# cortes-ciriano-lab/DeMethify

Measured on AMD Instinct MI355X. Metric: NMF update iters/sec (1e6 CpG x 256 samples x 16 types), higher is better.
Workload: dtype f64; 1 GPU; headline_1e6x256_12+4; N_cpg=1000000, S_samples=256, n_known=12, n_unknown=4, inner_iters=20, restarts=64, restart_seed=1 + k, restart_placement=k mod n_gpus, parallelism=restart-sharded x1

## Files before the change

demethify_amd/_lib.py:

```python
from __future__ import annotations

import ctypes as C
from pathlib import Path

LIB_PATH = Path(__file__).resolve().parent / "libdemethify_hip.so"

DMF_OK = 0
DMF_PTR_DEVICE = 1
DMF_INIT_IN_UNIT_RANGE = 4
DMF_SELECT_COUNTS_F32_EXACT, DMF_SELECT_PURITY, DMF_SELECT_ALPHA_OUTSIDE_UNIT, DMF_SELECT_V_UNALIGNED = 1, 2, 4, 8
DMF_SELECT_X16 = 16
DMF_COUNTS_F64 = 2
DMF_WLS_TARGET_V, DMF_WLS_TARGET_DV = 0, 1
DMF_WLS_F64_ARRAYS = 8
DMF_ERR_BAD_ARG, DMF_ERR_NONFINITE, DMF_ERR_UNSUPPORTED = 1, 4, 5
DMF_ERR_BAD_SHAPE = 2
DMF_GRAM_INTEGER, DMF_GRAM_FP64, DMF_GRAM_LAST = 0, 1, 2
DMF_ROUTE_SOLVER, DMF_ROUTE_UPDATE_U = 0, 1
MOMENTUM_SCALARS = ("a1", "a2", "l_w", "l_w_prev", "l_h", "l_h_prev", "dsq", "rt_norm2", "u_norm2", "cf", "cf_prev",
                    "iters", "done", "arrive", "mom_n", "mom_i")
REPORT_INTS = ("N", "S", "n_c", "ND", "SD", "N16", "plane_stride", "has_D16", "has_X16", "has_W16", "has_Dt8", "has_mask_bits",
               "rtp_width", "rtp_borrows_rt", "n_test", "d_f32_exact")
REPORT_DBLS = ("kDsq", "kRtSumsq", "kDmax", "kF32ResidualMax", "kIntCountMax", "kRtOutsideUnit", "x16_dev", "x16_sum")
PROBLEM_ARRAYS = {"V": 0, "D": 1, "Rt": 2, "Rtp": 3, "D16": 4, "X16": 5, "W16": 6, "Dt8": 7, "mask_bits": 8, "consts": 9}
DMF_MODE_PARTIAL = 0
DMF_MODE_UNSUPERVISED = 1
MAX_K = 64
SMALL_MAX_S, SMALL_MAX_K, SMALL_MAX_NU, SMALL_MAX_ELEMENTS = 64, 16, 4, 1 << 20
SVD_MAX_S, SVD_MAX_NC, SVD_MAX_RANK, SVD_MAX_LDS = 512, 64, 64, 160 * 1024


def svd_project_lds_bytes(n_samples, rank):
    return 8 * (n_samples * rank + 8 * ((n_samples + 63) // 64 * 64 + 16) + 512)


KERNEL_ROWPASS, KERNEL_GRAM, KERNEL_ALPHA, KERNEL_COST = 0, 1, 2, 3
KERNEL_FAMILIES = ("rowpass", "gram", "alpha", "cost")

_p = C.c_void_p
_i64 = C.c_int64
_dbl_p = C.POINTER(C.c_double)

SIGNATURES = {
    "dmf_status_string": (C.c_char_p, [C.c_int]),
    "dmf_last_error": (C.c_char_p, []),
    "dmf_abi_version": (C.c_int, []),
    "dmf_context_create": (C.c_int, [C.c_int, _p, C.POINTER(_p)]),
    "dmf_context_destroy": (C.c_int, [_p]),
    "dmf_context_synchronize": (C.c_int, [_p]),
    "dmf_context_set_profiling": (C.c_int, [_p, C.c_int]),
    "dmf_context_kernel_time": (C.c_int, [_p, C.c_int, _dbl_p, C.POINTER(_i64)]),
    "dmf_context_reset_kernel_time": (C.c_int, [_p]),
    "dmf_context_set_generic": (C.c_int, [_p, C.c_int]),
    "dmf_context_set_x16": (C.c_int, [_p, C.c_int]),
    "dmf_context_set_rowpass_pair": (C.c_int, [_p, C.c_int]),
    "dmf_context_set_rowpass_defer_c": (C.c_int, [_p, C.c_int]),
    "dmf_context_set_stop_confirmation": (C.c_int, [_p, C.c_int]),
    "dmf_problem_create": (C.c_int, [_p, _i64, _i64, _i64, _p, _p, _p, C.c_int, C.POINTER(_p)]),
    "dmf_problem_gather": (C.c_int, [_p, _p, _p, _i64, C.POINTER(_p)]),
    "dmf_problem_gather_device": (C.c_int, [_p, _p, _p, _i64, C.POINTER(_p)]),
    "dmf_problem_mask": (C.c_int, [_p, _p, _p, C.c_int, C.POINTER(_p)]),
    "dmf_solver_holdout_error": (C.c_int, [_p, _p, _dbl_p, C.POINTER(_i64)]),
    "dmf_problem_destroy": (C.c_int, [_p]),
    "dmf_problem_shape": (C.c_int, [_p, C.POINTER(_i64), C.POINTER(_i64), C.POINTER(_i64)]),
    "dmf_problem_gram_known": (C.c_int, [_p, _p, C.c_char_p, _i64]),
    "dmf_problem_report": (C.c_int, [_p, C.POINTER(_i64), _dbl_p]),
    "dmf_problem_copy_out": (C.c_int, [_p, C.c_int, _p, _i64]),
    "dmf_gram_i8_describe": (C.c_int, [_i64, _i64, _i64, _i64, C.c_int, C.c_char_p, _i64]),
    "dmf_solver_gram": (C.c_int, [_p, C.c_int, _p, C.c_char_p, _i64]),
    "dmf_solver_row_moments": (C.c_int, [_p, _p, C.c_char_p, _i64]),
    "dmf_solver_momentum_state": (C.c_int, [_p, _dbl_p, _p, _p]),
    "dmf_cost": (C.c_int, [_p, _p, _p, _i64, _p, C.c_int, _dbl_p]),
    "dmf_cost_describe": (C.c_int, [_i64, _i64, _i64, C.c_int, _i64, C.c_int, C.c_int, C.c_int, C.c_char_p, _i64]),
    "dmf_problem_cost_describe": (C.c_int, [_p, _p, _i64, C.c_char_p, _i64]),
    "dmf_project_simplex": (C.c_int, [_p, _p, _i64, _i64, C.c_double, C.c_int, _p]),
    "dmf_update_u": (C.c_int, [_p, _p, _p, _p, _p, _i64, _i64, C.c_int, C.c_int, _dbl_p, _p, _p]),
    "dmf_update_alpha": (C.c_int, [_p, _p, _p, _i64, _p, _p, _i64, C.c_int, _dbl_p, _p, _p]),
    "dmf_wls_intercept": (C.c_int, [_p, _p, _p, _i64, C.c_int, C.c_int, _p, C.POINTER(C.c_int)]),
    "dmf_wls_moments": (C.c_int, [_p, _p, _p, _i64, C.c_int, C.c_int, _p]),
    "dmf_nnls_normal": (C.c_int, [_p, _p, _p, _i64, _i64, _p, C.POINTER(C.c_int)]),
    "dmf_svd_gram": (C.c_int, [_p, _p, _p, C.c_int, _p, C.POINTER(_i64)]),
    "dmf_svd_factor": (C.c_int, [_p, _p, _p, _p, _i64, C.c_int, _p, C.POINTER(_p)]),
    "dmf_svd_finish": (C.c_int, [_p, _p, _i64, _i64, _p, _p, C.c_int, _p]),
    "dmf_percentile_axis0": (C.c_int, [_p, _p, _i64, _i64, _p, _i64, C.c_int, _p]),
    "dmf_nanpercentile_axis0": (C.c_int, [_p, _p, _i64, _i64, _p, _i64, C.c_int, _p]),
    "dmf_solver_create": (C.c_int, [_p, _p, _p, _p, _i64, C.c_int, C.c_int, C.POINTER(_p)]),
    "dmf_solver_set_purity": (C.c_int, [_p, _p, C.c_int]),
    "dmf_solver_step": (C.c_int, [_p, _i64, _i64, C.c_double, C.POINTER(_i64), C.POINTER(C.c_int)]),
    "dmf_solver_get": (C.c_int, [_p, C.c_int, _p, _p, _dbl_p, C.POINTER(_i64)]),
    "dmf_solver_match_components": (C.c_int, [_p, _p, _i64, _p, _p]),
    "dmf_solver_get_u_permuted": (C.c_int, [_p, C.POINTER(C.c_int32), _p]),
    "dmf_solver_get_u_by_row": (C.c_int, [_p, _p, _i64, C.POINTER(C.c_int32), _p]),
    "dmf_solver_cost": (C.c_int, [_p, _dbl_p]),
    "dmf_solver_cost_begin": (C.c_int, [_p]),
    "dmf_solver_cost_end": (C.c_int, [_p, _dbl_p]),
    "dmf_solver_destroy": (C.c_int, [_p]),
    "dmf_solver_describe": (C.c_int, [_p, _i64, C.c_char_p, _i64]),
    "dmf_select_describe": (C.c_int, [_i64, _i64, _i64, _i64, C.c_int, C.c_int, _i64, C.c_int, C.c_char_p, _i64]),
    "dmf_u_phase_describe": (C.c_int, [_i64, _i64, _i64, _i64, C.c_int, C.c_int, _i64, C.c_int, C.c_int, C.c_char_p, _i64]),
    "dmf_solver_u_phase_describe": (C.c_int, [_p, _i64, C.c_int, C.c_char_p, _i64]),
    "dmf_solver_stop_info": (C.c_int, [_p, C.POINTER(C.c_int), C.POINTER(_i64), C.POINTER(_i64), _dbl_p]),
    "dmf_solver_rowpass_launches": (C.c_int, [_p, C.POINTER(_i64), C.POINTER(_i64)]),
    "dmf_solver_rowpass_schedule_counts": (C.c_int, [_p, C.POINTER(_i64), C.POINTER(_i64), C.POINTER(_i64)]),
    "dmf_table_scan": (C.c_int, [C.c_char_p, C.c_char, C.POINTER(_i64), C.POINTER(C.c_int), C.POINTER(C.c_int),
                                 C.POINTER(C.c_int)]),
    "dmf_table_read": (C.c_int, [C.c_char_p, C.c_char, C.c_int, C.c_int, _i64, _p, _i64, C.c_double, _p, _i64, C.c_int]),
    "dmf_host_alloc": (_p, [C.c_size_t, C.POINTER(C.c_int)]),
    "dmf_host_free": (None, [_p, C.c_int]),
    "dmf_write_interval_csv": (C.c_int, [C.c_char_p, C.c_char_p, _p, _p, _i64, C.c_int, C.c_int, C.c_int]),
    "dmf_stage_upload": (C.c_int, [_p, _p, C.c_size_t, C.POINTER(C.c_void_p)]),
    "dmf_stage_free": (C.c_int, [_p, _p]),
    "dmf_stage_download": (C.c_int, [_p, _p, C.c_size_t, _p]),
    "dmf_mask_draw": (C.c_int, [_p, _p, C.POINTER(C.c_int), _i64, _i64, C.c_uint64, C.POINTER(C.c_void_p),
                                C.POINTER(_i64)]),
    "dmf_solve": (C.c_int, [_p, _p, _p, _p, _i64, C.c_int, _i64, _i64, C.c_double, C.c_int, _p, _p,
                            _dbl_p, C.POINTER(_i64)]),
    "dmf_solve_small_supported": (C.c_int, [_i64, _i64, _i64, _i64, C.c_int]),
    "dmf_solve_small": (C.c_int, [_p, _p, _i64, _p, _p, _p, _i64, C.c_int, _i64, _i64, C.c_double, _i64, C.c_int, _p, _p, _p, _p]),
    "dmf_solve_small_purity": (C.c_int, [_p, _p, _i64, _p, _p, _p, _p, _i64, C.c_int, _i64, _i64, C.c_double, _i64, C.c_int, _p, _p,
                                         _p, _p]),
}

_lib = None


class DemethifyHipError(RuntimeError):

    def __init__(self, status: int, where: str, detail: str = ""):
        self.status = status
        msg = f"{where}: status {status}"
        if detail:
            msg += f" ({detail})"
        super().__init__(msg)


def _preload_torch_hip_runtime():
    import importlib.util
    import os

# ... 48 lines not shown
```

demethify_amd/csrc/dmf_api.h:

```cpp
#pragma once
#include <hip/hip_runtime.h>

#include <cmath>
#include <cstdio>
#include <cstdlib>
#include <cstring>
#include <memory>
#include <mutex>
#include <new>
#include <unordered_map>
#include <utility>
#include <vector>

#include "../../include/demethify_hip.h"
#include "dmf_internal.h"
#include "dmf_select.h"

using dmf::SolverState;

namespace dmf_api {

int hip_fail(hipError_t e, const char* what, const char* file, int line);

#define HIP_TRY(expr)                                                                          \
    do {                                                                                       \
        hipError_t e_ = (expr);                                                                \
        if (e_ != hipSuccess) return dmf_api::hip_fail(e_, #expr, __FILE_NAME__, __LINE__);    \
    } while (0)

#define DMF_TRY(expr)                 \
    do {                              \
        int s_ = (expr);              \
        if (s_ != DMF_OK) return s_;  \
    } while (0)

constexpr int kEventPool = 2048;

struct FamilyClock {
    std::vector<hipEvent_t> start, stop;
    int used = 0;
    double total_ms = 0.0;
    int64_t launches = 0;
};

}

struct dmf_context {
    int device = 0;
    hipStream_t stream = nullptr;
    bool own_stream = false;
    unsigned profiling = 0;
    int stop_confirmation = 0;
    int generic_level = 0;
    bool x16 = true;
    bool rowpass_pair = true;
    bool rowpass_defer_c = true;
    double* scratch = nullptr;
    hipMemPool_t pool = nullptr;
    std::unordered_map<void*, size_t> live;
    std::unordered_map<size_t, std::vector<void*>> kept;
    size_t kept_bytes = 0;
    std::vector<hipEvent_t> events;
    std::vector<double*> pinned_moms;
    std::vector<void*> pinned_states;
    hipStream_t copy_stream = nullptr;
    std::mutex copy_mutex;
    dmf_api::FamilyClock clocks[DMF_KERNEL_FAMILIES];
};

namespace dmf_api {

hipError_t pool_alloc(dmf_context* ctx, void** p, size_t bytes);
void pool_free(dmf_context* ctx, void* p);
hipError_t stage_alloc(dmf_context* ctx, hipStream_t st, void** p, size_t bytes);
void stage_release(dmf_context* ctx, hipStream_t st, void* p);

template <class T>
class DevBuf {
  public:
    DevBuf() = default;
    DevBuf(DevBuf&& o) noexcept : ctx_(o.ctx_), ptr_(o.ptr_), owned_(o.owned_), stage_(o.stage_) {
        o.ptr_ = nullptr, o.owned_ = false;
    }
    DevBuf& operator=(DevBuf&& o) noexcept {
        if (this != &o) {
            reset();
            ctx_ = o.ctx_, ptr_ = o.ptr_, owned_ = o.owned_, stage_ = o.stage_;
            o.ptr_ = nullptr, o.owned_ = false;
        }
        return *this;
    }
    ~DevBuf() { reset(); }
    hipError_t alloc(dmf_context* ctx, size_t count) {
        reset();
        const hipError_t e = pool_alloc(ctx, (void**)&ptr_, count * sizeof(T));
        if (e != hipSuccess) ptr_ = nullptr;
        ctx_ = ctx, owned_ = e == hipSuccess, stage_ = nullptr;
        return e;
    }
    hipError_t alloc_staged(dmf_context* ctx, size_t count, hipStream_t st) {
        reset();
        const hipError_t e = stage_alloc(ctx, st, (void**)&ptr_, count * sizeof(T));
        if (e != hipSuccess) ptr_ = nullptr;
        ctx_ = ctx, owned_ = e == hipSuccess, stage_ = st;
        return e;
    }
    T* release() {
        T* p = ptr_;
        ptr_ = nullptr, owned_ = false;
        return p;
    }
    void borrow(const T* p) { reset(), ptr_ = const_cast<T*>(p); }
    void reset() {
        if (owned_ && stage_ != nullptr) stage_release(ctx_, stage_, ptr_);
        else if (owned_) pool_free(ctx_, ptr_);
        ptr_ = nullptr, owned_ = false;
    }
    T* get() const { return ptr_; }
    operator T*() const { return ptr_; }
    T* operator->() const { return ptr_; }

  private:
    dmf_context* ctx_ = nullptr;
    T* ptr_ = nullptr;
    bool owned_ = false;
    hipStream_t stage_ = nullptr;
};

enum ProblemConst { kDsq, kRtSumsq, kDmax, kF32ResidualMax, kIntCountMax, kRtOutsideUnit, kProblemConsts };

struct JobTable {
    std::vector<short> h_k, h_l;
    std::vector<int> h_dst;
    DevBuf<short> k, l;
    DevBuf<int> dst;
    int n = 0;
    template <class Keep>
    void build(int l_first, int l_last, Keep keep) {
        for (int ll = l_first; ll <= l_last; ++ll)
            for (int kk = 0; kk <= ll; ++kk) {
                if (!keep(kk, ll)) continue;
                h_k.push_back((short)kk);
                h_l.push_back((short)ll);
                h_dst.push_back(dmf::tri(kk, ll));
            }
        n = (int)h_k.size();
    }
    int upload(dmf_context* ctx) {
        HIP_TRY(k.alloc(ctx, n));
        HIP_TRY(l.alloc(ctx, n));
        HIP_TRY(dst.alloc(ctx, n));
        HIP_TRY(hipMemcpyAsync(k, h_k.data(), n * sizeof(short), hipMemcpyHostToDevice, ctx->stream));
        HIP_TRY(hipMemcpyAsync(l, h_l.data(), n * sizeof(short), hipMemcpyHostToDevice, ctx->stream));
        HIP_TRY(hipMemcpyAsync(dst, h_dst.data(), n * sizeof(int), hipMemcpyHostToDevice, ctx->stream));
        return DMF_OK;
    }
};

}

struct dmf_problem {
    dmf_context* ctx = nullptr;
    int64_t N = 0, S = 0, n_c = 0;
    dmf_api::DevBuf<double> V, D, Rt;
    dmf_api::DevBuf<double> Rtp;
    dmf_api::DevBuf<double> consts;
    double h_consts[dmf_api::kProblemConsts] = {};
    dmf_api::DevBuf<unsigned short> D16;
    dmf_api::DevBuf<signed char> Dt8;
    int ND = 0;
    int SD = 0;
    int64_t N16 = 0, plane_stride = 0;
    dmf_api::DevBuf<unsigned short> X16;
    double x16_dev = 0.0, x16_sum = 0.0;
    bool d_f32_exact = false;
    dmf_api::DevBuf<double> gb_known;
    dmf::GramRan known_ran;
    dmf_api::DevBuf<unsigned char> mask_bits;
    dmf_api::DevBuf<unsigned short> W16;
    int64_t n_test = 0;
    dmf::ProblemView view() const {
        dmf::ProblemView v;
        v.V = V, v.D = D, v.D16 = D16, v.X16 = X16, v.Dt8 = Dt8;
        v.plane_stride = plane_stride, v.SD = SD, v.ND = ND;
        v.Rt = Rt, v.Rtp = Rtp;
        v.N = N, v.S = (int)S, v.n_c = (int)n_c;
        return v;
    }
};

constexpr size_t kPinnedStateBytes = (sizeof(SolverState) + 15) / 16 * 16 + 16;

struct dmf_solver {
    dmf_context* ctx = nullptr;
    const dmf_problem* p = nullptr;
    int64_t n_u = 0;
    int mode = 0;
    dmf::ShapeKey key;
    dmf::PathSpec spec;
    dmf_api::DevBuf<double> cm;
    dmf_api::DevBuf<double> beta_tab;
    int64_t beta_cap = 0;
    dmf_api::DevBuf<long long> slab_i8;
    int64_t slab_i8_words = 0;
    dmf_api::DevBuf<long long> acc_i8;
    dmf_api::DevBuf<double> purity;
    dmf_api::DevBuf<double> u2_partials;
    dmf_api::DevBuf<double> u, u_prev, u_next;
    dmf_api::DevBuf<double> alpha, alpha_prev;
    dmf_api::DevBuf<double> gb;
    dmf::GramRan last_gram;
    int last_gram_source = -1;
    dmf_api::DevBuf<double> slab;
    int64_t slab_doubles = 0;
    dmf_api::DevBuf<double> partials;
    dmf_api::DevBuf<SolverState> state;
    SolverState* h_state = nullptr;
    dmf_api::JobTable jobs;
    bool cf_pending = true;
    double* mom_host = nullptr;
    dmf_api::DevBuf<double> mom_dev;
    hipEvent_t cost_event = nullptr;
    bool cost_pending = false;
    bool in_flight = false;
    bool confirm_stops = false;
    double cf_stream = 0.0;
    long long cf_stream_iter = -1;
    long long n_rowpass = 0, n_rowpass_pair = 0;
    long long n_rowpass_defer = 0;
    long long n_confirmed = 0, n_unconfirmed = 0;
    dmf::IterateView iterate() const {
        dmf::IterateView it;
        it.u = u, it.u_prev = u_prev, it.alpha = alpha, it.state = state;
        it.n_u = (int)n_u, it.mode = mode;
        return it;
    }
    dmf::AlphaView alpha_view() const {
        dmf::AlphaView a;
        a.gb = gb, a.alpha = alpha, a.alpha_prev = alpha_prev, a.purity = purity, a.state = state, a.partials = partials;
        a.S = (int)p->S, a.n_c = (int)p->n_c, a.n_u = (int)n_u;
        return a;
    }
    dmf::UScratch scratch() const {
        dmf::UScratch sc;
        sc.cm = cm, sc.beta = beta_tab, sc.slab = slab, sc.u2_partials = u2_partials;
        return sc;
    }
};

namespace dmf_api {

struct HandleDeleter {
    void operator()(dmf_problem* p) const { dmf_problem_destroy(p); }
    void operator()(dmf_solver* s) const { dmf_solver_destroy(s); }
};
using ProblemPtr = std::unique_ptr<dmf_problem, HandleDeleter>;
using SolverPtr = std::unique_ptr<dmf_solver, HandleDeleter>;

int clock_drain(dmf_context* ctx, FamilyClock& c);

struct FamilyScope {
    dmf_context* ctx;
    FamilyClock* c = nullptr;
    int slot = -1;
    FamilyScope(dmf_context* ctx_, int family) : ctx(ctx_) {
        if (!((ctx->profiling >> family) & 1u)) return;
        c = &ctx->clocks[family];
        if (c->start.empty()) {
            c->start.resize(kEventPool);
            c->stop.resize(kEventPool);
            for (int i = 0; i < kEventPool; ++i) {
                hipEventCreateWithFlags(&c->start[i], hipEventDisableSystemFence);
                hipEventCreateWithFlags(&c->stop[i], hipEventDisableSystemFence);
            }
        }
        if (c->used == kEventPool) clock_drain(ctx, *c);
        slot = c->used++;
        hipEventRecord(c->start[slot], ctx->stream);
    }
    ~FamilyScope() {
        if (c != nullptr) hipEventRecord(c->stop[slot], ctx->stream);
    }
};

int check_ctx(dmf_context* ctx);

template <class T>
int import_array(dmf_context* ctx, const void* src, size_t count, int flags, DevBuf<T>& dst) {
    dst.reset();
    if (count == 0) return DMF_OK;
    if (flags & DMF_PTR_DEVICE) {
        dst.borrow(static_cast<const T*>(src));
        return DMF_OK;
    }
    HIP_TRY(dst.alloc(ctx, count));
    HIP_TRY(hipMemcpyAsync(dst, src, count * sizeof(T), hipMemcpyHostToDevice, ctx->stream));
    HIP_TRY(hipStreamSynchronize(ctx->stream));
    return DMF_OK;
}
int export_array(dmf_context* ctx, const void* dev_src, size_t bytes, int flags, void* dst);

hipError_t enqueue_cost(dmf_context* ctx, const dmf::ProblemView& p, const double* u, const double* alpha, int n_u,
                        double* scratch, double* out);
bool cost_reads_u16_only(dmf_context* ctx, const dmf::ProblemView& p, int n_u);
int cost_to_host(dmf_context* ctx, const dmf::ProblemView& p, const double* u, const double* alpha, int n_u,
                 double* host_slot, bool wait);

int enqueue_u_phase(dmf_solver* s, int n_iter2, dmf::RowKind row);
dmf::RowKind standalone_row_kind(const dmf_solver* s, int n_iter2);
int enqueue_gram(dmf_solver* s, dmf::GramKind kind, bool heed_done = true, dmf::GramRan* ran = nullptr);
dmf::GramKind fp64_gram_kind(const dmf_solver* s);
int enqueue_alpha_phase(dmf_solver* s, dmf::AlphaKind kind, int n_iter2);
// ... 5 lines not shown
```

demethify_amd/csrc/dmf_api_context.hip:

```cpp
#include "dmf_api.h"

namespace dmf_api {

static thread_local char g_last_error[512] = "";

int hip_fail(hipError_t e, const char* what, const char* file, int line) {
    snprintf(g_last_error, sizeof(g_last_error), "%s failed at %s:%d: %s", what, file, line, hipGetErrorString(e));
    return DMF_ERR_HIP;
}

int clock_drain(dmf_context* ctx, FamilyClock& c) {
    if (c.used == 0) return DMF_OK;
    HIP_TRY(hipStreamSynchronize(ctx->stream));
    for (int i = 0; i < c.used; ++i) {
        float ms = 0.f;
        HIP_TRY(hipEventElapsedTime(&ms, c.start[i], c.stop[i]));
        c.total_ms += ms;
    }
    c.launches += c.used;
    c.used = 0;
    return DMF_OK;
}

static bool pool_enabled() {
// ... 218 lines not shown
    HIP_TRY(state.alloc_staged(ctx, kStateWords, st));
    uint32_t h_state[kStateWords] = {};
    std::memcpy(h_state, key, 624 * sizeof(uint32_t));
    HIP_TRY(hipMemcpyAsync(state, h_state, sizeof(h_state), hipMemcpyHostToDevice, st));
    HIP_TRY(dmf::launch_mask_draw(state, *pos, N, S, threshold, bits, reinterpret_cast<unsigned long long*>(state + 624), st));
    HIP_TRY(hipMemcpyAsync(h_state, state, sizeof(h_state), hipMemcpyDeviceToHost, st));
    HIP_TRY(hipStreamSynchronize(st));
    unsigned long long result[2];
    std::memcpy(result, h_state + 624, sizeof(result));
    std::memcpy(key, h_state, 624 * sizeof(uint32_t));
    *pos = (int)result[1];
    *n_kept = (int64_t)result[0];
    *out_bits = bits.release();
    return DMF_OK;
}

int dmf_stage_free(dmf_context* ctx, void* dev) {
    if (ctx == nullptr) return DMF_ERR_BAD_ARG;
    if (dev == nullptr) return DMF_OK;
    HIP_TRY(hipSetDevice(ctx->device));
    pool_free(ctx, dev);
    return DMF_OK;
}

int dmf_context_synchronize(dmf_context* ctx) {
    DMF_TRY(check_ctx(ctx));
    HIP_TRY(hipStreamSynchronize(ctx->stream));
    return DMF_OK;
}

int dmf_context_set_profiling(dmf_context* ctx, int enabled) {
    DMF_TRY(check_ctx(ctx));
    if (!enabled)
        for (auto& c : ctx->clocks) DMF_TRY(clock_drain(ctx, c));
    ctx->profiling = enabled == 0 ? 0u : enabled == 1 ? ~0u : (unsigned)enabled >> 1;
    return DMF_OK;
}

int dmf_context_kernel_time(dmf_context* ctx, int family, double* total_ms, int64_t* launches) {
    DMF_TRY(check_ctx(ctx));
    if (family < 0 || family >= DMF_KERNEL_FAMILIES) return DMF_ERR_BAD_ARG;
    FamilyClock& c = ctx->clocks[family];
    DMF_TRY(clock_drain(ctx, c));
    if (total_ms) *total_ms = c.total_ms;
    if (launches) *launches = c.launches;
    return DMF_OK;
}

int dmf_context_reset_kernel_time(dmf_context* ctx) {
    DMF_TRY(check_ctx(ctx));
    for (auto& c : ctx->clocks) {
        DMF_TRY(clock_drain(ctx, c));
        c.total_ms = 0.0;
        c.launches = 0;
    }
    return DMF_OK;
}

int dmf_context_set_generic(dmf_context* ctx, int enabled) {
    if (ctx == nullptr) return DMF_ERR_BAD_ARG;
    if (enabled < 0 || enabled > 4) return DMF_ERR_BAD_ARG;
    ctx->generic_level = enabled;
    return DMF_OK;
}

int dmf_context_set_x16(dmf_context* ctx, int enabled) {
    if (ctx == nullptr || enabled < 0 || enabled > 1) return DMF_ERR_BAD_ARG;
    ctx->x16 = enabled != 0;
    return DMF_OK;
}

int dmf_context_set_rowpass_pair(dmf_context* ctx, int enabled) {
    if (ctx == nullptr || enabled < 0 || enabled > 1) return DMF_ERR_BAD_ARG;
    ctx->rowpass_pair = enabled != 0;
    return DMF_OK;
}

int dmf_context_set_rowpass_defer_c(dmf_context* ctx, int enabled) {
    if (ctx == nullptr || enabled < 0 || enabled > 1) return DMF_ERR_BAD_ARG;
    ctx->rowpass_defer_c = enabled != 0;
    return DMF_OK;
}

int dmf_context_set_stop_confirmation(dmf_context* ctx, int mode) {
    if (ctx == nullptr || mode < 0 || mode > 2) return DMF_ERR_BAD_ARG;
    ctx->stop_confirmation = mode;
    return DMF_OK;
}

}
```

demethify_amd/csrc/dmf_api_problem.hip:

```cpp
#include "dmf_api.h"

namespace dmf_api {

static int alloc_count_copies(dmf_problem* p, int ND, bool x16, bool w16) {
    dmf_context* ctx = p->ctx;
    p->ND = ND;
    p->SD = (int)((p->S + 63) / 64 * 64);
    p->N16 = (p->N + 15) / 16 * 16;
    p->plane_stride = ((p->N + 31) / 32) * (p->SD / 32) * 1024;
    const size_t u16_elems = (size_t)p->N16 * p->SD;
    HIP_TRY(p->D16.alloc(ctx, u16_elems));
    HIP_TRY(p->Dt8.alloc(ctx, (size_t)p->plane_stride * ND));
    if (x16) HIP_TRY(p->X16.alloc(ctx, u16_elems));
    if (w16) HIP_TRY(p->W16.alloc(ctx, u16_elems));
    return DMF_OK;
}

static void known_route(dmf_problem* p, const char* piece) {
    char* t = p->known_ran.text;
    const size_t have = std::strlen(t), cap = sizeof(p->known_ran.text);
    snprintf(t + have, cap - have, "%s%s", have > 0 ? " " : "", piece);
}

static int problem_finalize(dmf_problem* p, bool counts_done = false) {
    dmf_context* ctx = p->ctx;
    const int64_t N = p->N, S = p->S, n_c = p->n_c;
    double* const h = p->h_consts;
    HIP_TRY(p->consts.alloc(ctx, kProblemConsts));
    if (!counts_done) HIP_TRY(dmf::launch_max_f64(p->D, N * S, ctx->scratch, p->consts + kDmax, ctx->stream));
    if (n_c > 0) {
        HIP_TRY(dmf::launch_sumsq_f64(p->Rt, N * n_c, ctx->scratch + 1024, p->consts + kRtSumsq, nullptr, ctx->stream));
    } else {
        HIP_TRY(hipMemsetAsync(p->consts + kRtSumsq, 0, sizeof(double), ctx->stream));
    }
    if (!counts_done) {
        HIP_TRY(dmf::launch_f32_residual_max(p->D, N * S, ctx->scratch + 2048, p->consts + kF32ResidualMax, ctx->stream));
        HIP_TRY(dmf::launch_int_count_max(p->D, N * S, ctx->scratch + 3072, p->consts + kIntCountMax, ctx->stream));
        if (n_c > 0) {
            HIP_TRY(dmf::launch_unit_range_check(p->Rt, N * n_c, ctx->scratch, p->consts + kRtOutsideUnit, ctx->stream));
        } else {
            HIP_TRY(hipMemsetAsync(p->consts + kRtOutsideUnit, 0, sizeof(double), ctx->stream));
        }
    }
    {
        double got[kProblemConsts];
        HIP_TRY(hipMemcpyAsync(got, p->consts, sizeof(got), hipMemcpyDeviceToHost, ctx->stream));
        HIP_TRY(hipStreamSynchronize(ctx->stream));
        h[kRtSumsq] = got[kRtSumsq];
        if (!counts_done)
            for (int i = kDmax; i < kProblemConsts; ++i) h[i] = got[i];
    }
    h[kDsq] = h[kDmax] * h[kDmax];
    p->d_f32_exact = h[kF32ResidualMax] == 0.0;
    HIP_TRY(hipMemcpyAsync(p->consts, h, kProblemConsts * sizeof(double), hipMemcpyHostToDevice, ctx->stream));
    HIP_TRY(hipStreamSynchronize(ctx->stream));
    if (!std::isfinite(h[kDmax]) || !std::isfinite(h[kRtSumsq])) return DMF_ERR_NONFINITE;

    if (!counts_done && ctx->generic_level == 0 && h[kIntCountMax] <= 32639.0 && h[kRtOutsideUnit] == 0.0 && S >= 2 &&
        S <= 2048 && n_c <= 48) {
        DMF_TRY(alloc_count_copies(p, h[kIntCountMax] <= 127.0 ? 1 : 2, ctx->x16, false));
        DevBuf<unsigned long long> x_stats;
        if (ctx->x16) HIP_TRY(x_stats.alloc(ctx, 3));
        HIP_TRY(dmf::launch_build_counts_int(p->D, p->V, N, (int)S, p->ND, p->D16, p->X16, p->N16, p->SD, p->Dt8,
                                             p->plane_stride, x_stats, ctx->stream));
        if (p->X16 != nullptr) {
            unsigned long long got[3] = {1, 0, 0};
            HIP_TRY(hipMemcpyAsync(got, x_stats, sizeof(got), hipMemcpyDeviceToHost, ctx->stream));
            HIP_TRY(hipStreamSynchronize(ctx->stream));
            if (got[0] != 0) {
                p->X16.reset();
            } else {
                std::memcpy(&p->x16_dev, &got[1], sizeof(double));
                p->x16_sum = (double)got[2];
            }
        }
    }

    if (n_c > 0 && n_c <= 48) {
        const int nct = (int)((n_c + 3) / 4 * 4);
        if (nct == n_c) {
            p->Rtp.borrow(p->Rt);
        } else {
            HIP_TRY(p->Rtp.alloc(ctx, (size_t)N * nct));
            HIP_TRY(dmf::launch_pad_rows(p->Rt, p->Rtp, N, (int)n_c, nct, ctx->stream));
        }
    }

    const dmf::ProblemView pv = p->view();
    JobTable jobs;
    jobs.build(0, (int)n_c, [](int, int) { return true; });
    const int n_jobs = jobs.n;
    const bool mfma = n_c >= 1 && ctx->generic_level != 1 && ctx->generic_level != 2;
    const int n_fast = mfma ? n_jobs - 1 : 0, n_dense = (int)(n_c * (n_c + 1) / 2);
    const bool int_known = mfma && ctx->generic_level == 0 && p->Dt8 != nullptr && p->D16 != nullptr && p->Rtp != nullptr &&
                           (reinterpret_cast<uintptr_t>(p->Rtp.get()) & 15) == 0 &&
                           dmf::gram_i8_known_supported((int)n_c, p->ND, N, p->SD);
    int64_t slab_doubles = dmf::gram_slab_doubles(N, (int)S, mfma ? 1 : n_jobs);
    if (mfma && !int_known) {
        const int64_t need = dmf::gram_mfma_slab_doubles(N, (int)S, n_fast);
        if (need > slab_doubles) slab_doubles = need;
    }
    DevBuf<double> slab, slab_bu;
    DevBuf<long long> slab_i8, acc;
    HIP_TRY(p->gb_known.alloc(ctx, (size_t)n_jobs * S));
    DMF_TRY(jobs.upload(ctx));
    HIP_TRY(slab.alloc(ctx, (size_t)slab_doubles));
    bool vdv_done = true;
    if (int_known) {
        const int64_t slab_words = dmf::gram_i8_slab_words_nf(N, p->SD, n_dense);
        const int64_t acc_words = dmf::gram_i8_acc_words_nf((int)S, n_dense, (int)n_c + 1);
        HIP_TRY(slab_i8.alloc(ctx, (size_t)slab_words));
        HIP_TRY(acc.alloc(ctx, (size_t)acc_words));
        HIP_TRY(slab_bu.alloc(ctx, (size_t)dmf::bu_cols_grid(N) * (n_c + 1) * S));
        HIP_TRY(hipMemsetAsync(acc, 0, (size_t)acc_words * sizeof(long long), ctx->stream));
        int ny = 0, n_slabs = 0;
        dmf::GramRan ran;
        HIP_TRY(dmf::launch_gram_i8(pv, nullptr, 0, jobs.k, jobs.l, n_dense, slab_i8, slab_words, nullptr, &ny, ctx->stream, &ran));
        known_route(p, "int_known");
        known_route(p, ran.text);
        HIP_TRY(dmf::launch_bu_cols(pv, p->Rt, (int)n_c, slab_bu, nullptr, &n_slabs, ctx->stream, &vdv_done));
        known_route(p, vdv_done ? "+ k_bu_cols2 with vDv" : "+ k_bu_cols");
        HIP_TRY(dmf::launch_gram_v2_reduce(slab_i8, ny, n_dense, p->SD, slab_bu, n_slabs, (int)n_c + (vdv_done ? 1 : 0), (int)S,
                                           acc, jobs.dst, p->gb_known, nullptr, nullptr, 0, nullptr, ctx->stream));
    } else if (mfma) {
        dmf::GramJobTable fast{jobs.k, jobs.l, jobs.dst, n_fast};
        int ny = 0;
        dmf::GramRan ran;
        HIP_TRY(dmf::launch_gram_mfma(pv, nullptr, 0, fast, n_dense, slab, slab_doubles, nullptr, &ny, ctx->stream, &ran));
        known_route(p, "fp64");
        known_route(p, ran.text);
        HIP_TRY(dmf::launch_gram_reduce(slab, ny, n_fast, (int)S, jobs.dst, p->gb_known, nullptr, ctx->stream));
    }
    if (int_known && vdv_done) {
    } else if (n_jobs - n_fast == 1 && ctx->generic_level != 1 && ctx->generic_level != 2 &&
               (int64_t)dmf::vdv_cols_grid(N) * S <= slab_doubles) {
        HIP_TRY(dmf::launch_vdv_cols(pv, slab, p->gb_known + (int64_t)jobs.h_dst[n_jobs - 1] * S, ctx->stream));
        known_route(p, p->known_ran.text[0] == 0 ? "fp64 k_vdv_cols" : "+ k_vdv_cols");
    } else {
        dmf::GramJobTable rest{jobs.k + n_fast, jobs.l + n_fast, jobs.dst + n_fast, n_jobs - n_fast};
        dmf::GramRan ran;
        if (p->known_ran.text[0] == 0) known_route(p, "fp64");
        else known_route(p, "+");
        HIP_TRY(dmf::launch_gram(pv, nullptr, 0, rest, slab, slab_doubles, p->gb_known, nullptr, ctx->stream, &ran));
        known_route(p, ran.text);
    }
    HIP_TRY(hipStreamSynchronize(ctx->stream));
    return DMF_OK;
}

static dmf::CostPlan cost_plan_of(dmf_context* ctx, const dmf::ProblemView& p, int n_u) {
    return dmf::cost_plan(dmf::cost_key(p, n_u, ctx->generic_level));
}

hipError_t enqueue_cost(dmf_context* ctx, const dmf::ProblemView& p, const double* u, const double* alpha, int n_u,
                        double* scratch, double* out) {
    return dmf::launch_cost_plan(cost_plan_of(ctx, p, n_u), p, u, alpha, n_u, scratch, out, ctx->stream);
}

bool cost_reads_u16_only(dmf_context* ctx, const dmf::ProblemView& p, int n_u) { return cost_plan_of(ctx, p, n_u).d16; }
// ... 148 lines not shown
    const bool x16 = ints && src->X16 != nullptr && ctx->x16;
    if (ints) DMF_TRY(alloc_count_copies(p.get(), src->ND, x16, true));
    DevBuf<unsigned long long> d_stats;
    HIP_TRY(d_stats.alloc(ctx, 3));
    HIP_TRY(dmf::launch_mask_problem(src->V, src->D, ints ? src->D16.get() : nullptr, x16 ? src->X16.get() : nullptr,
                                     p->mask_bits, p->V, p->D, p->D16, p->X16, p->W16, N, p->N16, (int)S, p->SD, d_stats,
                                     ctx->stream));
    if (ints) HIP_TRY(dmf::launch_build_dt8(p->D16, N, p->SD, p->ND, p->Dt8, p->plane_stride, ctx->stream));
    unsigned long long h_stats[3] = {0, 0, 0};
    HIP_TRY(hipMemcpyAsync(h_stats, d_stats, sizeof(h_stats), hipMemcpyDeviceToHost, ctx->stream));
    HIP_TRY(hipStreamSynchronize(ctx->stream));
    d_stats.reset();
    double dmax;
    std::memcpy(&dmax, &h_stats[0], sizeof(dmax));
    p->h_consts[kDmax] = dmax;
    p->h_consts[kF32ResidualMax] = src->h_consts[kF32ResidualMax];
    p->h_consts[kIntCountMax] = std::isfinite(src->h_consts[kIntCountMax]) ? dmax : src->h_consts[kIntCountMax];
    p->h_consts[kRtOutsideUnit] = src->h_consts[kRtOutsideUnit];
    p->x16_dev = x16 ? src->x16_dev : 0.0;
    p->x16_sum = (double)h_stats[1];
    p->n_test = (int64_t)h_stats[2];
    DMF_TRY(problem_finalize(p.get(), true));
    *out = p.release();
    return DMF_OK;
}

int dmf_problem_destroy(dmf_problem* p) {
    if (p == nullptr) return DMF_OK;
    hipSetDevice(p->ctx->device);
    delete p;
    return DMF_OK;
}

int dmf_problem_cost_describe(dmf_context* ctx, const dmf_problem* p, int64_t n_u, char* buf, int64_t cap) {
    if (ctx == nullptr || p == nullptr || buf == nullptr || cap < 1 || n_u < 0 || p->ctx != ctx) return DMF_ERR_BAD_ARG;
    if (p->n_c + n_u < 1 || p->n_c + n_u > dmf::kMaxK) return DMF_ERR_BAD_ARG;
    dmf::describe_cost_plan(cost_plan_of(ctx, p->view(), (int)n_u), buf, (size_t)cap);
    return DMF_OK;
}

int dmf_problem_gram_known(const dmf_problem* p, double* out, char* out_text, int64_t cap) {
    if (p == nullptr || out == nullptr || (out_text != nullptr && cap < 1)) return DMF_ERR_BAD_ARG;
    dmf_context* ctx = p->ctx;
    DMF_TRY(check_ctx(ctx));
    const size_t n = (size_t)(p->n_c + 1) * (p->n_c + 2) / 2 * p->S;
    HIP_TRY(hipMemcpyAsync(out, p->gb_known, n * sizeof(double), hipMemcpyDeviceToHost, ctx->stream));
    HIP_TRY(hipStreamSynchronize(ctx->stream));
    if (out_text != nullptr) snprintf(out_text, (size_t)cap, "%s", p->known_ran.text);
    return DMF_OK;
}

int dmf_problem_report(const dmf_problem* p, int64_t* out_ints, double* out_dbls) {
    if (p == nullptr || out_ints == nullptr || out_dbls == nullptr) return DMF_ERR_BAD_ARG;
    const int64_t rtp_width = p->Rtp != nullptr ? (p->n_c + 3) / 4 * 4 : 0;
    const int64_t ints[DMF_REPORT_INTS] = {p->N, p->S, p->n_c, p->ND, p->SD, p->N16, p->plane_stride,
                                           p->D16 != nullptr, p->X16 != nullptr, p->W16 != nullptr, p->Dt8 != nullptr,
                                           p->mask_bits != nullptr, rtp_width,
                                           p->Rtp != nullptr && p->Rtp.get() == p->Rt.get(), p->n_test, p->d_f32_exact};
    std::memcpy(out_ints, ints, sizeof(ints));
    for (int i = 0; i < kProblemConsts; ++i) out_dbls[i] = p->h_consts[i];
    out_dbls[kProblemConsts] = p->x16_dev;
    out_dbls[kProblemConsts + 1] = p->x16_sum;
    return DMF_OK;
}

int dmf_problem_copy_out(const dmf_problem* p, int which, void* out, int64_t bytes) {
    if (p == nullptr || out == nullptr) return DMF_ERR_BAD_ARG;
    dmf_context* ctx = p->ctx;
    DMF_TRY(check_ctx(ctx));
    const size_t elems = (size_t)p->N * p->S, u16_bytes = (size_t)p->N16 * p->SD * sizeof(unsigned short);
    const void* src = nullptr;
    size_t size = 0;
    switch (which) {
        case DMF_ARRAY_V: src = p->V, size = elems * sizeof(double); break;
        case DMF_ARRAY_D: src = p->D, size = elems * sizeof(double); break;
        case DMF_ARRAY_RT: src = p->Rt, size = (size_t)p->N * p->n_c * sizeof(double); break;
        case DMF_ARRAY_RTP: src = p->Rtp, size = (size_t)p->N * ((p->n_c + 3) / 4 * 4) * sizeof(double); break;
        case DMF_ARRAY_D16: src = p->D16, size = u16_bytes; break;
        case DMF_ARRAY_X16: src = p->X16, size = u16_bytes; break;
        case DMF_ARRAY_W16: src = p->W16, size = u16_bytes; break;
        case DMF_ARRAY_DT8: src = p->Dt8, size = (size_t)p->plane_stride * p->ND; break;
        case DMF_ARRAY_MASK_BITS: src = p->mask_bits, size = (size_t)p->N * (size_t)((p->S + 7) / 8); break;
        case DMF_ARRAY_CONSTS: src = p->consts, size = kProblemConsts * sizeof(double); break;
        default: return DMF_ERR_BAD_ARG;
    }
    if (src == nullptr || size == 0) return DMF_ERR_BAD_ARG;
    if (bytes < 0 || (size_t)bytes != size) return DMF_ERR_BAD_SHAPE;
    return export_array(ctx, src, size, 0, out);
}

int dmf_problem_shape(const dmf_problem* p, int64_t* N, int64_t* S, int64_t* n_c) {
    if (p == nullptr) return DMF_ERR_BAD_ARG;
    if (N) *N = p->N;
    if (S) *S = p->S;
    if (n_c) *n_c = p->n_c;
    return DMF_OK;
}

}
```

demethify_amd/csrc/dmf_api_solver.hip:

```cpp
#include "dmf_api.h"

namespace dmf_api {

using dmf::kSplitInnerSteps;

static int ensure_split_scratch(dmf_solver* s, int n_iter2) {
    dmf_context* ctx = s->ctx;
    if (s->cm == nullptr) HIP_TRY(s->cm.alloc(ctx, (size_t)dmf::u_phase_split_cm_doubles(s->p->N, (int)s->n_u)));
    if (s->beta_cap < n_iter2 || s->beta_tab == nullptr) {
        s->beta_cap = n_iter2 > 0 ? n_iter2 : 1;
        HIP_TRY(s->beta_tab.alloc(ctx, (size_t)s->beta_cap));
    }
    return DMF_OK;
}

int enqueue_u_phase(dmf_solver* s, int n_iter2, dmf::RowKind row) {
    dmf_context* ctx = s->ctx;
    const dmf::ProblemView pv = s->p->view();
    FamilyScope scope(ctx, DMF_KERNEL_ROWPASS);
    switch (row) {
        case dmf::RowKind::CmI8InnerRows:
            DMF_TRY(ensure_split_scratch(s, n_iter2));
            HIP_TRY(dmf::launch_u_phase_split_i8(pv, s->iterate(), n_iter2, s->scratch(), ctx->stream));
            return DMF_OK;
// ... 41 lines not shown
    return b;
}

static int gram_i8_and_reduce(dmf_solver* s, const GramI8Buffers& b, int n_slabs, const double* u2_partials, int n_u2,
                              dmf::GramRan* ran = nullptr) {
    dmf_context* ctx = s->ctx;
    const dmf_problem* p = s->p;
    const int S = (int)p->S, n_c = (int)p->n_c, n_u = (int)s->n_u, nf = n_c * n_u + n_u * (n_u + 1) / 2;
    int ny = 0;
    HIP_TRY(dmf::launch_gram_i8(p->view(), s->u, n_u, s->jobs.k, s->jobs.l, nf, b.slab_i8, b.slab_i8_words, b.done, &ny,
                                ctx->stream, ran));
    HIP_TRY(dmf::launch_gram_v2_reduce(b.slab_i8, ny, nf, p->SD, b.slab_bu, n_slabs, n_u, S, b.acc, s->jobs.dst, b.gb, b.done,
                                       u2_partials, n_u2, s->state, ctx->stream));
    return DMF_OK;
}

static int gram_bu_cols_i8(dmf_solver* s, const GramI8Buffers& b, dmf::GramRan* ran = nullptr) {
    int n_slabs = 0;
    HIP_TRY(dmf::launch_bu_cols(s->p->view(), s->u, (int)s->n_u, b.slab_bu, b.done, &n_slabs, s->ctx->stream));
    return gram_i8_and_reduce(s, b, n_slabs, nullptr, 0, ran);
}

int enqueue_gram(dmf_solver* s, dmf::GramKind kind, bool heed_done, dmf::GramRan* ran) {
    dmf_context* ctx = s->ctx;
    const dmf::ProblemView pv = s->p->view();
    const int S = pv.S, n_u = (int)s->n_u;
    const int* done = heed_done ? &s->state->done : nullptr;
    FamilyScope scope(ctx, DMF_KERNEL_GRAM);
    if (kind == dmf::GramKind::BuColsI8) {
        GramI8Buffers b = solver_i8_buffers(s);
        b.done = done;
        return gram_bu_cols_i8(s, b, ran);
    }
    if (kind == dmf::GramKind::GramU) {
        int ny = 0;
        HIP_TRY(dmf::launch_gram_u(pv, s->u, n_u, s->slab, done, &ny, ctx->stream, ran));
        HIP_TRY(dmf::launch_gram_reduce(s->slab, ny, s->jobs.n, S, s->jobs.dst, s->gb, done, ctx->stream));
        return DMF_OK;
    }
    dmf::GramJobTable jobs{s->jobs.k, s->jobs.l, s->jobs.dst, s->jobs.n};
    if (kind == dmf::GramKind::GramMfma) {
        int ny = 0;
        HIP_TRY(dmf::launch_gram_mfma(pv, s->u, n_u, jobs, s->jobs.n - n_u, s->slab, s->slab_doubles, done, &ny, ctx->stream, ran));
        HIP_TRY(dmf::launch_gram_reduce(s->slab, ny, s->jobs.n, S, s->jobs.dst, s->gb, done, ctx->stream));
        return DMF_OK;
    }
    HIP_TRY(dmf::launch_gram(pv, s->u, n_u, jobs, s->slab, s->slab_doubles, s->gb, done, ctx->stream, ran));
    return DMF_OK;
}

dmf::GramKind fp64_gram_kind(const dmf_solver* s) {
    return s->spec.use_gram_spec ? dmf::GramKind::GramU : s->spec.use_gram_mfma ? dmf::GramKind::GramMfma : dmf::GramKind::Gram;
}

int enqueue_alpha_phase(dmf_solver* s, dmf::AlphaKind kind, int n_iter2) {
    FamilyScope scope(s->ctx, DMF_KERNEL_ALPHA);
    HIP_TRY(dmf::launch_alpha(kind, s->alpha_view(), n_iter2, s->ctx->stream));
    return DMF_OK;
}

constexpr int kLastGramI8Tail = 100, kLastGramFused = 101;
static dmf::GramRan* last_gram_slot(dmf_solver* s, int source) {
    if (s->last_gram_source == source) return nullptr;
    s->last_gram_source = source;
    return &s->last_gram;
}

static int enqueue_gram_i8_tail(dmf_solver* s, dmf::AlphaKind alpha, int n_iter2, int grid) {
    {
        FamilyScope scope(s->ctx, DMF_KERNEL_GRAM);
        DMF_TRY(gram_i8_and_reduce(s, solver_i8_buffers(s), grid, s->u2_partials, grid, last_gram_slot(s, kLastGramI8Tail)));
    }
    return enqueue_alpha_phase(s, alpha, n_iter2);
}

static int enqueue_outer_iteration(dmf_solver* s, int n_iter2) {
    dmf_context* ctx = s->ctx;
    s->in_flight = true;
    const dmf_problem* p = s->p;
    const int S = (int)p->S;
    const dmf::IterationPlan plan = dmf::plan_iteration(s->key, s->spec, n_iter2, s->purity != nullptr);
    if (plan.row == dmf::RowKind::RowpassV2) {
        int grid = 0;
        bool paired = false, deferred = false;
        {
            FamilyScope scope(ctx, DMF_KERNEL_ROWPASS);
            dmf::ProblemView pv = p->view();
            if (!s->key.x16) pv.X16 = nullptr;
            HIP_TRY(dmf::launch_rowpass_v2(pv, s->iterate(), n_iter2, s->scratch(), &grid, s->key.rowpass_pair, &paired,
                                           s->key.rowpass_defer_c && s->key.x_byte, &deferred, ctx->stream));
            ++s->n_rowpass;
            s->n_rowpass_pair += paired ? 1 : 0;
            s->n_rowpass_defer += deferred ? 1 : 0;
        }
        return enqueue_gram_i8_tail(s, plan.alpha, n_iter2, grid);
    }
    if (plan.row == dmf::RowKind::CmI8InnerBu) {
        int grid = 0;
        DMF_TRY(ensure_split_scratch(s, n_iter2));
        {
            FamilyScope scope(ctx, DMF_KERNEL_ROWPASS);
            HIP_TRY(dmf::launch_u_phase_split_i8_bu(p->view(), s->iterate(), n_iter2, s->scratch(), &grid, ctx->stream));
        }
        return enqueue_gram_i8_tail(s, plan.alpha, n_iter2, grid);
    }
    if (plan.row == dmf::RowKind::RowpassFused) {
        const int64_t n_full = p->N - (p->N & 15), n_tail = p->N - n_full;
        const dmf::ProblemView pv = p->view();
        int grid = 0, ny_tail = 0;
        {
            FamilyScope scope(ctx, DMF_KERNEL_ROWPASS);
            HIP_TRY(dmf::launch_rowpass_fused(pv.rows(0, n_full), s->iterate(), n_iter2, s->scratch(), &grid, ctx->stream));
        }
        if (n_tail > 0) {
            const dmf::ProblemView tail = pv.rows(n_full, n_tail);
            const dmf::IterateView it_tail = s->iterate().rows(n_full);
            HIP_TRY(dmf::launch_u_phase_mfma(tail, it_tail, n_iter2, ctx->stream));
            HIP_TRY(dmf::launch_sumsq_f64(it_tail.u, n_tail * s->n_u, ctx->scratch, s->u2_partials + grid, &s->state->done,
                                          ctx->stream));
            HIP_TRY(dmf::launch_gram_u(tail, it_tail.u, it_tail.n_u, s->slab + (int64_t)2 * grid * s->jobs.n * S,
                                       &s->state->done, &ny_tail, ctx->stream));
        }
        if (dmf::GramRan* ran = last_gram_slot(s, kLastGramFused))
            snprintf(ran->text, sizeof(ran->text), "k_rowpass_fused<%d,%d> phase C slabs=%d%s", (int)(p->n_c + 3) / 4, (int)s->n_u,
                     2 * grid, n_tail > 0 ? " + k_gram_u tail" : "");
        HIP_TRY(dmf::launch_finish_u_norm(s->u2_partials, grid + (n_tail > 0 ? 1 : 0), s->state, ctx->stream));
        {
            FamilyScope scope(ctx, DMF_KERNEL_GRAM);
            HIP_TRY(dmf::launch_gram_reduce(s->slab, 2 * grid + ny_tail, s->jobs.n, S, s->jobs.dst, s->gb,
                                            &s->state->done, ctx->stream));
        }
        return enqueue_alpha_phase(s, plan.alpha, n_iter2);
    }
    DMF_TRY(enqueue_u_phase(s, n_iter2, plan.row));
    HIP_TRY(dmf::launch_sumsq_f64(s->u, p->N * s->n_u, ctx->scratch, &s->state->u_norm2, &s->state->done,
                                  ctx->stream));
    HIP_TRY(dmf::launch_set_lh(s->state, ctx->stream));
    DMF_TRY(enqueue_gram(s, plan.gram, true, last_gram_slot(s, (int)plan.gram)));
    return enqueue_alpha_phase(s, plan.alpha, n_iter2);
}

int fetch_state(dmf_solver* s) {
    HIP_TRY(hipMemcpyAsync(s->h_state, s->state, sizeof(SolverState), hipMemcpyDeviceToHost, s->ctx->stream));
    HIP_TRY(hipStreamSynchronize(s->ctx->stream));
    s->in_flight = false;
    return DMF_OK;
}

int push_state(dmf_solver* s) {
    HIP_TRY(hipMemcpyAsync(s->state, s->h_state, sizeof(SolverState), hipMemcpyHostToDevice, s->ctx->stream));
    HIP_TRY(hipStreamSynchronize(s->ctx->stream));
    return DMF_OK;
}

constexpr int kMomRows = 64, kMomSteps = 64;

__global__ void k_set_momentum(SolverState* state, const double* mom, int stride, int rows, int n) {
    state->mom = mom;
    state->mom_stride = stride;
    state->mom_rows = rows;
    state->mom_i = 0;
    state->mom_n = n;
}

static double momentum_advance(double& a) {
#pragma clang fp contract(off)
    const double a0 = a;
    const double sq = 4.0 * a0 * a0;
    a = (1.0 + std::sqrt(1.0 + sq)) / 2.0;
    return (a0 - 1.0) / a;
}

static int upload_momentum_rows(dmf_solver* s, int rows, int n) {
    dmf_context* ctx = s->ctx;
    const int stride = 2 + 2 * n;
    if (s->mom_host == nullptr) {
        if (!ctx->pinned_moms.empty()) {
            s->mom_host = ctx->pinned_moms.back();
            ctx->pinned_moms.pop_back();
        } else {
            HIP_TRY(hipHostMalloc((void**)&s->mom_host, (size_t)kMomRows * (2 + 2 * kMomSteps) * sizeof(double)));
        }
        HIP_TRY(s->mom_dev.alloc(ctx, (size_t)kMomRows * (2 + 2 * kMomSteps)));
    }
    double a1 = s->h_state->a1, a2 = s->h_state->a2;
    for (int r = 0; r < rows; ++r) {
        double* row = s->mom_host + (size_t)r * stride;
        for (int t = 0; t < n; ++t) {
            row[2 + t] = momentum_advance(a1);
            row[2 + n + t] = momentum_advance(a2);
        }
        row[0] = a1;
        row[1] = a2;
    }
    HIP_TRY(hipMemcpyAsync(s->mom_dev, s->mom_host, (size_t)rows * stride * sizeof(double), hipMemcpyHostToDevice, ctx->stream));
    hipLaunchKernelGGL(k_set_momentum, dim3(1), dim3(1), 0, ctx->stream, s->state.get(), (const double*)s->mom_dev.get(), stride,
                       rows, n);
    HIP_TRY(hipGetLastError());
    return DMF_OK;
}

__global__ void k_set_tol(SolverState* state, double tol, double band) {
    state->tol = tol;
    state->band = band;
}

constexpr double kConfirmBand = 10.0;
constexpr double kGramCostRelErr = 1e-15;

static double* cost_slot(const dmf_solver* s) {
    return reinterpret_cast<double*>(reinterpret_cast<char*>(s->h_state) + kPinnedStateBytes - 16);
}

static int solver_setup(dmf_solver* s, const double* u0, const double* alpha0, int flags) {
    dmf_context* ctx = s->ctx;
    const dmf_problem* p = s->p;
    const int64_t N = p->N, S = p->S, n_c = p->n_c, n_u = s->n_u, K = n_c + n_u;
    dmf::ShapeKey& key = s->key;
    key.N = N;
    key.S = (int)S;
    key.n_c = (int)n_c;
    key.n_u = (int)n_u;
    key.nd = (p->ND > 0 && p->D16 != nullptr) ? p->ND : 0;
    key.SD = p->SD;
    key.x16 = key.nd > 0 && p->X16 != nullptr;
    key.rowpass_pair = ctx->rowpass_pair;
    key.rowpass_defer_c = ctx->rowpass_defer_c;
    key.x_byte = key.x16 && p->h_consts[kIntCountMax] <= 255.0;
    key.level = ctx->generic_level;
    key.d_f32_exact = p->d_f32_exact;
    key.rtp_present = n_c == 0 || p->Rtp != nullptr;
    key.v_align = (unsigned)(reinterpret_cast<uintptr_t>(p->V.get()) & 15);
    key.rtp_align = (unsigned)(reinterpret_cast<uintptr_t>(p->Rtp.get()) & 15);
    key.alpha_unit = true;
    s->spec = dmf::select_path(key);
    if ((s->spec.use_v2 || s->spec.use_cm_i8) && !(flags & DMF_INIT_IN_UNIT_RANGE)) {
        bool in_unit = true;
        if (flags & DMF_PTR_DEVICE) {
            double outside = 0.0;
            HIP_TRY(dmf::launch_unit_range_check(alpha0, K * S, ctx->scratch, ctx->scratch + 2048, ctx->stream));
            HIP_TRY(hipMemcpyAsync(&outside, ctx->scratch + 2048, sizeof(double), hipMemcpyDeviceToHost, ctx->stream));
            HIP_TRY(hipStreamSynchronize(ctx->stream));
            in_unit = outside == 0.0;
        } else {
            for (int64_t i = 0; i < K * S; ++i)
                if (!(alpha0[i] >= 0.0 && alpha0[i] <= 1.0)) {
                    in_unit = false;
                    break;
                }
        }
        if (!in_unit) {
            key.alpha_unit = false;
            s->spec = dmf::select_path(key);
        }
    }
    if (!s->spec.supported) return DMF_ERR_UNSUPPORTED;
    s->in_flight = true;
    s->jobs.build((int)n_c, (int)K, [n_c, K](int k, int l) {
        if (l == (int)K && k < (int)n_c) return false;
        return !(l == (int)K && k == (int)K);
    });
    const int n_jobs = s->jobs.n;
    s->slab_doubles = dmf::gram_slab_doubles(N, (int)S, n_jobs);
    if (s->spec.use_gram_spec) {
        const int64_t spec = dmf::gram_u_slab_doubles(N, (int)S, (int)n_c, (int)n_u);
        if (spec > s->slab_doubles) s->slab_doubles = spec;
    }
    if (s->spec.use_gram_mfma) {
        const int64_t need = dmf::gram_mfma_slab_doubles(N, (int)S, n_jobs);
        if (need > s->slab_doubles) s->slab_doubles = need;
    }
    if (s->spec.use_fused) {
        const int64_t spec = dmf::rowpass_fused_slab_doubles(N - (N & 15), (int)S, (int)n_c, (int)n_u) +
                             dmf::gram_u_slab_doubles(16, (int)S, (int)n_c, (int)n_u);
        if (spec > s->slab_doubles) s->slab_doubles = spec;
    }
    if (s->spec.use_v2) {
        const int64_t bu = (int64_t)dmf::rowpass_v2_grid(N, (int)S) * n_u * S;
        if (bu > s->slab_doubles) s->slab_doubles = bu;
    }
    if (s->spec.use_gram_i8) {
        const int64_t bu = (int64_t)dmf::bu_cols_grid(N) * n_u * S;
        if (bu > s->slab_doubles) s->slab_doubles = bu;
        if (s->spec.use_cm_i8) {
            const int64_t bu2 = (int64_t)dmf::u_inner_bu_grid(N, (int)S) * n_u * S;
            if (bu2 > s->slab_doubles) s->slab_doubles = bu2;
        }
    }
    const size_t un = (size_t)N * n_u, an = (size_t)K * S;
    const size_t un_alloc = (un + 1) & ~(size_t)1;
    const size_t gbn = (size_t)(K + 1) * (K + 2) / 2 * S;
    const int nb_alpha = (int)((S + 63) / 64);
    HIP_TRY(s->u.alloc(ctx, un_alloc));
    HIP_TRY(s->u_prev.alloc(ctx, un_alloc));
    if (s->spec.u_path == 2) HIP_TRY(s->u_next.alloc(ctx, un_alloc));
    HIP_TRY(s->alpha.alloc(ctx, an));
    HIP_TRY(s->alpha_prev.alloc(ctx, an));
    HIP_TRY(s->gb.alloc(ctx, gbn));
    HIP_TRY(s->slab.alloc(ctx, (size_t)s->slab_doubles));
    HIP_TRY(s->partials.alloc(ctx, (size_t)2 * (nb_alpha + S)));
    HIP_TRY(s->u2_partials.alloc(ctx, 4096));
    if (s->spec.use_v2 || s->spec.use_gram_i8) {
        s->slab_i8_words = dmf::gram_i8_slab_words(N, p->SD, (int)n_c, (int)n_u);
        HIP_TRY(s->slab_i8.alloc(ctx, (size_t)s->slab_i8_words));
        const size_t acc_words = (size_t)dmf::gram_i8_acc_words((int)S, (int)n_c, (int)n_u);
        HIP_TRY(s->acc_i8.alloc(ctx, acc_words));
        HIP_TRY(hipMemsetAsync(s->acc_i8, 0, acc_words * sizeof(long long), ctx->stream));
    }
    HIP_TRY(s->state.alloc(ctx, 1));
    if (!ctx->pinned_states.empty()) {
// ... 277 lines not shown
    if (s->h_state->done != 0) return DMF_ERR_BAD_ARG;
    dmf::CmRan ran;
    s->in_flight = true;
    const int status = solver_row_moments_enqueue(s, row, out_cm, &ran);
    if (status != DMF_OK) (void)hipStreamSynchronize(ctx->stream);
    s->in_flight = false;
    if (status == DMF_OK && out_text != nullptr) snprintf(out_text, (size_t)cap, "%s", ran.text);
    return status;
}

int dmf_solver_momentum_state(const dmf_solver* s, double* scalars, double* alpha_prev, double* u_prev) {
    if (s == nullptr || scalars == nullptr) return DMF_ERR_BAD_ARG;
    dmf_context* ctx = s->ctx;
    DMF_TRY(check_ctx(ctx));
    const dmf_problem* p = s->p;
    SolverState st;
    HIP_TRY(hipMemcpyAsync(&st, s->state.get(), sizeof(SolverState), hipMemcpyDeviceToHost, ctx->stream));
    if (alpha_prev != nullptr)
        HIP_TRY(hipMemcpyAsync(alpha_prev, s->alpha_prev.get(), (size_t)(p->n_c + s->n_u) * p->S * sizeof(double), hipMemcpyDeviceToHost,
                               ctx->stream));
    if (u_prev != nullptr)
        HIP_TRY(hipMemcpyAsync(u_prev, s->u_prev.get(), (size_t)p->N * s->n_u * sizeof(double), hipMemcpyDeviceToHost, ctx->stream));
    HIP_TRY(hipStreamSynchronize(ctx->stream));
    const double out[DMF_MOMENTUM_SCALARS] = {st.a1, st.a2, st.l_w, st.l_w_prev, st.l_h, st.l_h_prev, st.dsq, st.rt_norm2,
                                              st.u_norm2, st.cf, st.cf_prev, (double)st.iters, (double)st.done,
                                              (double)st.arrive, (double)st.mom_n, (double)st.mom_i};
    for (int i = 0; i < DMF_MOMENTUM_SCALARS; ++i) scalars[i] = out[i];
    return DMF_OK;
}

int dmf_solver_destroy(dmf_solver* s) {
    if (s == nullptr) return DMF_OK;
    dmf_context* ctx = s->ctx;
    hipSetDevice(ctx->device);
    if (s->cost_pending) (void)hipEventSynchronize(s->cost_event);
    if (s->in_flight) (void)hipStreamSynchronize(ctx->stream);
    if (s->cost_event) ctx->events.push_back(s->cost_event);
    if (s->mom_host) ctx->pinned_moms.push_back(s->mom_host);
    if (s->h_state) ctx->pinned_states.push_back(s->h_state);
    delete s;
    return DMF_OK;
}

int dmf_solver_describe(const dmf_solver* s, int64_t n_iter2, char* buf, int64_t cap) {
    if (s == nullptr || buf == nullptr || cap < 1 || n_iter2 < 0) return DMF_ERR_BAD_ARG;
    const dmf::IterationPlan plan = dmf::plan_iteration(s->key, s->spec, (int)n_iter2, s->purity != nullptr);
    dmf::describe_plan(s->key, plan, buf, (size_t)cap);
    return DMF_OK;
}

int dmf_solver_u_phase_describe(const dmf_solver* s, int64_t n_iter2, int route, char* buf, int64_t cap) {
    if (s == nullptr || buf == nullptr || cap < 1 || n_iter2 < 0 || n_iter2 > (1 << 20) ||
        (route != DMF_ROUTE_SOLVER && route != DMF_ROUTE_UPDATE_U))
        return DMF_ERR_BAD_ARG;
    dmf::describe_u_phase(s->key, s->spec, (int)n_iter2, s->purity != nullptr, route == DMF_ROUTE_UPDATE_U, buf, (size_t)cap);
    return DMF_OK;
}

int dmf_solver_stop_info(const dmf_solver* s, int* confirm_stops, int64_t* n_confirmed, int64_t* n_unconfirmed,
                         double* last_stream_cost) {
    if (s == nullptr) return DMF_ERR_BAD_ARG;
    if (confirm_stops) *confirm_stops = s->confirm_stops ? 1 : 0;
    if (n_confirmed) *n_confirmed = s->n_confirmed;
    if (n_unconfirmed) *n_unconfirmed = s->n_unconfirmed;
    if (last_stream_cost) *last_stream_cost = s->cf_stream_iter >= 0 ? s->cf_stream : std::nan("");
    return DMF_OK;
}

int dmf_solver_rowpass_launches(const dmf_solver* s, int64_t* total, int64_t* paired) {
    if (s == nullptr) return DMF_ERR_BAD_ARG;
    if (total) *total = s->n_rowpass;
    if (paired) *paired = s->n_rowpass_pair;
    return DMF_OK;
}

int dmf_solver_rowpass_schedule_counts(const dmf_solver* s, int64_t* total, int64_t* paired, int64_t* deferred) {
    if (s == nullptr) return DMF_ERR_BAD_ARG;
    if (total) *total = s->n_rowpass;
    if (paired) *paired = s->n_rowpass_pair;
    if (deferred) *deferred = s->n_rowpass_defer;
    return DMF_OK;
}

int dmf_solve(dmf_context* ctx, const dmf_problem* p, const double* u0, const double* alpha0, int64_t n_u,
              int mode, int64_t n_iter1, int64_t n_iter2, double tol, int flags, double* out_u,
              double* out_alpha, double* out_cost, int64_t* out_iters) {
    dmf_solver* raw = nullptr;
    DMF_TRY(dmf_solver_create(ctx, p, u0, alpha0, n_u, mode, flags, &raw));
    SolverPtr s(raw);
    DMF_TRY(dmf_solver_step(raw, n_iter1, n_iter2, tol, nullptr, nullptr));
    return dmf_solver_get(raw, flags, out_u, out_alpha, out_cost, out_iters);
}

}
```

demethify_amd/csrc/dmf_internal.h:

```cpp
#pragma once
#include <hip/hip_runtime.h>
#include <stdint.h>

#include "dmf_select.h"

namespace dmf {

struct SolverState {
    double a1;
    double a2;
    double l_w;
    double l_w_prev;
    double l_h;
    double l_h_prev;
    double dsq;
    double rt_norm2;
    double u_norm2;
    double cf;
    double cf_prev;
    double tol;
    long long iters;
    double band;
    int done;
    int arrive;
    const double* mom;
    int mom_stride, mom_rows, mom_i, mom_n;
};

__device__ __forceinline__ const double* momentum_row(const SolverState* __restrict__ state, int n_iter2) {
    return (state->mom != nullptr && state->mom_n == n_iter2 && state->mom_i < state->mom_rows)
               ? state->mom + (int64_t)state->mom_i * state->mom_stride
               : nullptr;
}

__host__ __device__ inline int tri(int k, int l) { return l * (l + 1) / 2 + k; }

constexpr int kMaxK = 64;
constexpr int kGramChunk = 16;
constexpr int kRowsPerBlockU = 64;

struct GramJobTable {
    const short* k_idx;
    const short* l_idx;
    const int* dst_row;
    int count;
};

struct PercentilePlan {
    long long k_prev, k_next;
    double gamma;
    int from_top;
    int pad;
};

struct ProblemView {
    const double* V = nullptr;
    const double* D = nullptr;
    const unsigned short* D16 = nullptr;
    const unsigned short* X16 = nullptr;
    const signed char* Dt8 = nullptr;
    int64_t plane_stride = 0;
    int SD = 0, ND = 0;
    const double* Rt = nullptr;
    const double* Rtp = nullptr;
    int64_t N = 0;
    int S = 0, n_c = 0;
    unsigned v_align() const { return (unsigned)(reinterpret_cast<uintptr_t>(V) & 15); }
    ProblemView rows(int64_t first, int64_t count) const {
        ProblemView r;
        r.V = V + first * S;
        r.D = D + first * S;
        r.Rt = Rt ? Rt + first * n_c : nullptr;
        r.Rtp = Rtp ? Rtp + first * ((n_c + 3) / 4 * 4) : nullptr;
        r.N = count;
        r.S = S;
        r.n_c = n_c;
        return r;
    }
};

struct IterateView {
    double* u = nullptr;
    double* u_prev = nullptr;
    const double* alpha = nullptr;
    SolverState* state = nullptr;
    int n_u = 0, mode = 0;
    IterateView rows(int64_t first) const {
        IterateView r = *this;
        r.u = u + first * n_u;
        r.u_prev = u_prev + first * n_u;
        return r;
    }
};

struct AlphaView {
    const double* gb = nullptr;
    double* alpha = nullptr;
    double* alpha_prev = nullptr;
    const double* purity = nullptr;
    SolverState* state = nullptr;
    double* partials = nullptr;
    int S = 0, n_c = 0, n_u = 0;
};

struct UScratch {
    double* cm = nullptr;
    double* beta = nullptr;
    double* slab = nullptr;
    double* u2_partials = nullptr;
};


hipError_t launch_convert_counts(const long long* src, double* dst, int64_t n, hipStream_t st);
hipError_t launch_max_f64(const double* x, int64_t n, double* scratch, double* out, hipStream_t st);
hipError_t launch_f32_residual_max(const double* x, int64_t n, double* scratch, double* out, hipStream_t st);
hipError_t launch_int_count_max(const double* x, int64_t n, double* scratch, double* out, hipStream_t st);
hipError_t launch_unit_range_check(const double* x, int64_t n, double* scratch, double* out, hipStream_t st);
hipError_t launch_sumsq_f64(const double* x, int64_t n, double* scratch, double* out,
                            const int* done_flag, hipStream_t st);
hipError_t launch_pad_rows(const double* src, double* dst, int64_t n_rows, int width_src, int width_dst,
                           hipStream_t st);
hipError_t launch_index_range_check(const long long* idx, int64_t n_idx, int64_t n_src, unsigned int* flag, hipStream_t st);
hipError_t launch_gather_rows(const double* src, double* dst, const long long* idx, int64_t n_idx,
                              int64_t width, hipStream_t st);

inline CostKey cost_key(const ProblemView& p, int n_u, int level) {
    CostKey k;
    k.S = p.S, k.n_c = p.n_c, k.n_u = n_u;
    k.d16 = p.D16 != nullptr;
    k.SD = p.SD;
    k.v_align = p.v_align();
    k.rtp_present = p.Rtp != nullptr;
    k.level = level;
    return k;
}
hipError_t launch_cost_plan(const CostPlan& plan, const ProblemView& p, const double* u, const double* alpha, int n_u,
                            double* scratch, double* out, hipStream_t st);
int vdv_cols_grid(int64_t N);
hipError_t launch_vdv_cols(const ProblemView& p, double* slab, double* out, hipStream_t st);

struct GramRan {
    char text[192] = "";
// ... 62 lines not shown

hipError_t launch_alpha(AlphaKind kind, const AlphaView& a, int n_iter2, hipStream_t st);
hipError_t launch_set_lh(SolverState* state, hipStream_t st);
hipError_t launch_project_simplex(const double* X, double* out, int K, int S, double z,
                                  hipStream_t st);
hipError_t launch_scatter_known_block(const double* gb_known, double* gb, int n_c, int K, int S,
                                      hipStream_t st);
hipError_t launch_init_state(SolverState* state, const double* consts, const double* alpha,
                             int S, int n_c, int n_u, hipStream_t st);

int64_t u_phase_split_cm_doubles(int64_t N, int n_u);
hipError_t launch_u_phase_split(const ProblemView& p, const IterateView& it, int n_iter2, const UScratch& scratch,
                                hipStream_t st);

bool cm_i8_supported(unsigned v_align, int S, int n_c, int n_u, int ND, int SD);
struct CmI8Launch {
    int mt0 = 0, mt1 = 0;
    int c_tile = 0, c_store = 0;
    size_t lds = 0;
    int grid = 0;
    int64_t blocks_per_wave = 0;
};
struct CmI8Panel {
    int col0 = 0, Sp = 0;
    bool s4 = false;
    int ncgx = 2;
    int tpl = 0;
    int n_launch = 0;
    CmI8Launch first, last;
};
constexpr int kCmMaxPanels = 8;
struct CmI8Plan {
    bool supported = false;
    int64_t N = 0;
    int S = 0, n_c = 0, n_u = 0;
    int nkc = 0, nd = 1;
    int nmt = 0, n_ct = 0;
    int n_panels = 0;
    CmI8Panel panel[kCmMaxPanels];
};
CmI8Plan cm_i8_plan(int64_t N, int S, int n_c, int n_u, int ND);
CmI8Launch cm_i8_launch_of(const CmI8Plan& g, int panel, int li);
int describe_cm_i8_plan(const CmI8Plan& g, char* buf, size_t cap);
struct CmRan {
    char text[2048] = "";
};
hipError_t launch_cm_i8(const ProblemView& p, const IterateView& it, double* cm, hipStream_t st, CmRan* ran = nullptr);
hipError_t launch_u_phase_split_i8(const ProblemView& p, const IterateView& it, int n_iter2, const UScratch& scratch,
                                   hipStream_t st);

bool u_inner_bu_supported(unsigned v_align, int S, int SD, int n_u, int n_iter2);
int u_inner_bu_grid(int64_t N, int S);
hipError_t launch_u_phase_split_i8_bu(const ProblemView& p, const IterateView& it, int n_iter2, const UScratch& scratch,
                                      int* grid_out, hipStream_t st);

bool u_phase_big_supported(int S, int n_c, int n_u, int n_iter2);
hipError_t launch_u_phase_big(const ProblemView& p, const IterateView& it, int n_iter2, hipStream_t st);

hipError_t launch_gram_mfma(const ProblemView& p, const double* u, int n_u, GramJobTable jobs, int n_dense, double* slab,
                            int64_t slab_doubles, const int* done_flag, int* ny_out, hipStream_t st, GramRan* ran = nullptr);
int64_t gram_mfma_slab_doubles(int64_t N, int S, int n_jobs);

hipError_t launch_gather_counts_int(const unsigned short* src16, const unsigned short* src_x16, const long long* idx,
                                    int64_t n_idx, int SD, int ND, unsigned short* D16, unsigned short* X16, int64_t N16,
                                    signed char* Dt8, int64_t plane_stride, unsigned int* max_out,
                                    unsigned long long* xsum_out, hipStream_t st);
constexpr double kX16MaxDev = 8.0 * 0x1p-53;
hipError_t launch_build_counts_int(const double* D, const double* V, int64_t N, int S, int ND, unsigned short* D16,
                                   unsigned short* X16, int64_t N16, int SD, signed char* Dt8, int64_t plane_stride,
                                   unsigned long long* x_stats, hipStream_t st);
hipError_t launch_build_dt8(const unsigned short* D16, int64_t N, int SD, int ND, signed char* Dt8, int64_t plane_stride,
                            hipStream_t st);
hipError_t launch_mask_problem(const double* srcV, const double* srcD, const unsigned short* src16,
                               const unsigned short* srcX, const unsigned char* bits, double* dstV, double* dstD,
                               unsigned short* dst16, unsigned short* dstX, unsigned short* W16, int64_t N, int64_t N16, int S,
                               int SD, unsigned long long* stats, hipStream_t st);
hipError_t launch_holdout_weights_f64(const unsigned char* bits, double* W, int64_t N, int S, hipStream_t st);
constexpr int64_t kMaskDrawMaxS = ((int64_t)1 << 31) - 1, kMaskDrawMaxElements = (int64_t)1 << 60;
hipError_t launch_mask_draw(unsigned int* key_io, int pos, int64_t N, int64_t S, unsigned long long threshold,
                            unsigned char* bits, unsigned long long* result, hipStream_t st);
bool rowpass_v2_supported(int S, int n_c, int n_u, int n_iter2);
int rowpass_v2_grid(int64_t N, int S);
hipError_t launch_rowpass_v2(const ProblemView& p, const IterateView& it, int n_iter2, const UScratch& scratch, int* grid_out,
                             bool pair, bool* paired_out, bool defer_c, bool* deferred_out, hipStream_t st);
bool rowpass_v2_pair_fits(int S, int n_u, int n_iter2);
bool gram_i8_supported(int n_c, int n_u, int ND, int64_t N, int SD);
struct GramI8Plan {
    bool supported = false;
    int xl = 1, nd = 1, ring = 8;
    int nf = 0, launches = 0;
    int nsh = 0, ny = 0;
    int64_t rows_per_wg = 0;
    int blocks = 0, last = 0;
    int tail = 0;
    bool xcd = false;
};
GramI8Plan gram_i8_plan(int64_t N, int SD, int n_c, int n_u, int ND);
void describe_gram_i8_plan(const GramI8Plan& g, char* buf, size_t cap);
int64_t gram_i8_slab_words(int64_t N, int SD, int n_c, int n_u);
int64_t gram_i8_acc_words(int S, int n_c, int n_u);
bool gram_i8_known_supported(int n_c, int ND, int64_t N, int SD);
int64_t gram_i8_slab_words_nf(int64_t N, int SD, int nf);
int64_t gram_i8_acc_words_nf(int S, int nf, int n_bu);
hipError_t launch_gram_i8(const ProblemView& p, const double* u, int n_u, const short* feat_a, const short* feat_b, int NF,
                          long long* slab, int64_t slab_words, const int* done_flag, int* ny_out, hipStream_t st,
                          GramRan* ran = nullptr);
int bu_cols_grid(int64_t N);
hipError_t launch_bu_cols(const ProblemView& p, const double* u, int n_u, double* slab, const int* done_flag,
                          int* n_slabs_out, hipStream_t st, bool* with_vdv = nullptr);
hipError_t launch_gram_v2_reduce(const long long* slab_i8, int ny, int NF, int SD, const double* slab_bu, int n_bu_slabs,
                                 int n_u, int S, long long* acc_words, const int* dst_row, double* gb, const int* done_flag,
                                 const double* u2_partials, int n_u2, SolverState* state, hipStream_t st);

hipError_t launch_percentile_pair(const double* x, int64_t n, int64_t m, PercentilePlan p0, PercentilePlan p1,
                                  double* out0, double* out1, hipStream_t st);
hipError_t launch_nanpercentile_pair(const double* x, int64_t n, int64_t m, PercentilePlan p0, PercentilePlan p1, double q0,
                                     double q1, double* out0, double* out1, hipStream_t st);
int64_t percentile_max_replicates();

int wls_moments_grid(int64_t N);
int64_t wls_slab_doubles(int64_t N, int S, int K);
hipError_t launch_wls_moments(const ProblemView& p, const double* u, int n_u, int target_dv, double* slab, double* mom,
                              hipStream_t st);
hipError_t launch_nnls_intercept(const double* gb, const double* mom, int K, int S, double* out, int* status, hipStream_t st);

constexpr int kSvdMaxS = 512, kSvdMaxNc = 64, kSvdMaxRank = 64;
constexpr size_t kSvdMaxLds = 160 * 1024;
size_t svd_project_lds_bytes(int S, int rank);
struct SvdColumns {
    double sign[kSvdMaxRank], scale[kSvdMaxRank];
};
bool svd_supported(int S, int n_c, int rank);
int svd_gram_grid(int64_t N, int S);
int64_t svd_gram_slab_doubles(int64_t N, int S);
hipError_t launch_svd_gram(const ProblemView& p, const double* H1, double* slab, int* flags, double* C, hipStream_t st);
int64_t svd_project_slab_doubles(int64_t N, int rank);
hipError_t launch_svd_project(const ProblemView& p, const double* H1, const double* Es, int rank, double* T, double* slab,
                              double* norms, hipStream_t st);
hipError_t launch_svd_finish(double* T, int64_t N, int rank, const SvdColumns& cols, hipStream_t st);

struct MatchColumns {
    int src[kMaxK];
};
int match_gram_grid(int64_t N, int n_u);
int64_t match_gram_slab_doubles(int64_t N, int n_u);
hipError_t launch_match_gram(const double* u, const double* anchor, const long long* idx, int64_t N, int64_t n_anchor_rows,
                             int n_u, double* slab, int* flags, double* P, hipStream_t st);
hipError_t launch_copy_cols_permuted(const double* u, double* dst, int64_t N, int n_u, const MatchColumns& cols,
                                     hipStream_t st);
constexpr long long kNotDrawn = 0x7fffffffffffffffLL;
hipError_t launch_first_occurrence(const long long* idx, int64_t M, int64_t n_dst_rows, long long* first,
                                   unsigned long long* n_bad, hipStream_t st);
hipError_t launch_copy_rows_first(const double* u, const long long* first, double* dst, int64_t n_dst_rows, int n_u,
                                  const MatchColumns& cols, hipStream_t st);

}
```

demethify_amd/csrc/dmf_kernels_rowpass2.hip:

```cpp
#include "dmf_device.h"
#include "dmf_dispatch.h"
#include "dmf_internal.h"
#include "dmf_ustep.h"
#include "dmf_fixedpoint.h"
#include <cstdlib>
#include <type_traits>

namespace dmf {

typedef double v4d __attribute__((ext_vector_type(4)));
typedef double v2d __attribute__((ext_vector_type(2)));
typedef unsigned int v4u __attribute__((ext_vector_type(4)));
typedef unsigned int v2u __attribute__((ext_vector_type(2)));
typedef int v4i __attribute__((ext_vector_type(4)));

#ifdef DMF_STAMPS
#define DMF2_NSTAMP 20
#define DMF2_STAMP_DECL unsigned long long st_last = dmf2_stamp(), st_seg[DMF2_NSTAMP] = {0, 0, 0, 0, 0, 0, 0, 0, 0, 0, 0, 0, 0, 0, 0, 0, 0, 0, 0, 0};
#define DMF2_STAMP(i) { const unsigned long long st_now = dmf2_stamp(); st_seg[i] += st_now - st_last; st_last = st_now; }
#define DMF2_STAMP_FLUSH                                                                                        \
    st_seg[15] = __builtin_amdgcn_s_getreg(4 | (31 << 11));                                                     \
    if (lane == 0) for (int i_ = 0; i_ < DMF2_NSTAMP; ++i_) stamps_out[((size_t)blockIdx.x * 4 + wave) * DMF2_NSTAMP + i_] = st_seg[i_];
__device__ __forceinline__ unsigned long long dmf2_stamp() {
    unsigned long long t;
    __builtin_amdgcn_sched_barrier(0);
    asm volatile("s_memtime %0\n\ts_waitcnt lgkmcnt(0)" : "=s"(t)::"memory");
    __builtin_amdgcn_sched_barrier(0);
    return t;
}
#define DMF2_SUB_BEGIN unsigned long long st_sub = dmf2_stamp();
#define DMF2_SUB(i) { const unsigned long long st_now = dmf2_stamp(); st_seg[i] += st_now - st_sub; st_sub = st_now; }
#else
#define DMF2_STAMP_DECL
#define DMF2_STAMP(i)
#define DMF2_STAMP_FLUSH
#define DMF2_SUB_BEGIN
#define DMF2_SUB(i)
#endif

#ifndef DMF_V2_STAGGER
#define DMF_V2_STAGGER 12
#endif
#ifndef DMF_V2_DEFER_PRIO
#define DMF_V2_DEFER_PRIO 1
#endif
#ifndef DMF_V2_STAGGER_DEFER
#define DMF_V2_STAGGER_DEFER 0
#endif

namespace {
constexpr int kRowV = 66;
constexpr int kRowD = 72;
constexpr int kTileVBytes2 = 16 * kRowV * 8;
constexpr int kTileDBytes2 = 16 * kRowD * 2;
constexpr int kTileBytes2 = kTileVBytes2 + kTileDBytes2;
constexpr int kTileBytesX = 2 * kTileDBytes2;
constexpr int kRingBlockBytes = 16 * 64;
constexpr int kRingBytes = 6 * kRingBlockBytes;
constexpr int kDeferUbufSets = 6;
}

template <int NU, bool AT_PREV>
__device__ __forceinline__ void inner_steps(double& uu, double& up, double cj, const double (&Ms)[NU], int b_lo, int b_hi,
                                            int t_end, int lane0) {
    int t2 = 0;
    for (; t2 + 1 < t_end; t2 += 2) {
        inner_step<NU, AT_PREV>(uu, up, cj, Ms, b_lo, b_hi, t2, lane0);
        inner_step<NU, AT_PREV>(up, uu, cj, Ms, b_lo, b_hi, t2 + 1, lane0);
    }
    if (t2 < t_end) {
        inner_step<NU, AT_PREV>(uu, up, cj, Ms, b_lo, b_hi, t2, lane0);
        const double tmp = uu;
        uu = up;
        up = tmp;
    }
}

constexpr int kUnrolledSteps = 20;

template <int NU, bool AT_PREV>
__device__ __forceinline__ void inner_steps_unrolled(double& uu, double& up, double cj, const double (&Ms)[NU], int b_lo, int b_hi,
                                                     int lane0) {
    static_assert(kUnrolledSteps % 2 == 0 && kUnrolledSteps <= 64, "pairs of steps; beta_t in lane t of one register pair");
#pragma unroll
    for (int t2 = 0; t2 < kUnrolledSteps; t2 += 2) {
        inner_step<NU, AT_PREV>(uu, up, cj, Ms, b_lo, b_hi, t2, lane0);
        inner_step<NU, AT_PREV>(up, uu, cj, Ms, b_lo, b_hi, t2 + 1, lane0);
    }
}

template <int NKC, int NU, int MAXW = 4, bool XS = false, bool PAIR = false, bool DEFER_C = false>
__global__ __launch_bounds__(64 * MAXW, MAXW == 4 ? 2 : 1) void k_rowpass_v2(
    const double* __restrict__ V, const unsigned short* __restrict__ D16, const unsigned short* __restrict__ X16, int SD,
    const double* __restrict__ Rtp,
    const double* __restrict__ alpha, double* __restrict__ u, double* __restrict__ u_prev,
    const SolverState* __restrict__ state, int64_t N, int S, int n_c, int n_iter2, int mode, int nd,
    double* __restrict__ slab, double* __restrict__ u2_partials
#ifdef DMF_STAMPS
    , unsigned long long* __restrict__ stamps_out
#endif
    ) {
    static_assert(NU >= 1 && NU <= 4, "one phase-B pass per block, 4x4x4 MFMA for the c product");
    static_assert(!PAIR || (XS && MAXW == 4), "the pair schedule: X16 form, two workgroups per CU");
    static_assert(!DEFER_C || PAIR, "the deferred-C schedule is a pair schedule");
    constexpr int NSET = PAIR ? 2 : 1;
    constexpr int NUB = DEFER_C ? kDeferUbufSets : NSET;
    constexpr int NCT = 4 * NKC;
    constexpr int NP = NU * (NU + 1) / 2;
    constexpr int SLOT = (NU + 2) & ~1;
    constexpr int NV = NU * SLOT;
    extern __shared__ double lds_dyn[];
    if (state->done) return;

    const int NW = blockDim.x >> 6;
    const int wave = __builtin_amdgcn_readfirstlane(threadIdx.x >> 6);
    const int lane = threadIdx.x & 63;
    const int wcol0 = wave * 64;

    double* __restrict__ beta_tab = lds_dyn;
    double* __restrict__ ubuf = beta_tab + ((n_iter2 + 1) & ~1);
    double* __restrict__ red = ubuf + NUB * 16 * NU;
    double* __restrict__ u2red = red + NSET * MAXW * NV * 16;
    constexpr int TB = XS ? (DEFER_C ? kTileDBytes2 : kTileBytesX) : kTileBytes2;
    char* __restrict__ tile = reinterpret_cast<char*>(u2red + MAXW) + (size_t)wave * TB;
    struct BlockTile {
        double* V;
        unsigned short *D, *X;
    };
    auto block_tile = [&](int set) {
        char* const t = tile + (size_t)set * NW * TB;
        unsigned short* const d = reinterpret_cast<unsigned short*>(t + (XS ? 0 : kTileVBytes2));
        return BlockTile{reinterpret_cast<double*>(t), d, d + 16 * kRowD};
    };
    unsigned int* const ring = reinterpret_cast<unsigned int*>(tile + (size_t)(NSET * NW - wave) * TB + (size_t)wave * kRingBytes);
    auto ring_at = [&](int slot, int row, int dword) {
        return ring + slot * (kRingBlockBytes / 4) + (4 * (row & 3) + (row >> 2)) * 16 + ((dword + 4 * (row & 3)) & 15);
    };

    if (const double* __restrict__ mrow = momentum_row(state, n_iter2)) {
        const double lw_prev = state->l_w_prev, lw = state->l_w;
        for (int t2 = threadIdx.x; t2 < n_iter2; t2 += blockDim.x)
            beta_tab[t2] = fmin(mrow[2 + t2], t2 == 0 ? 0.9999 * sqrt(lw_prev / lw) : 0.9999);
    } else if (threadIdx.x == 0) {
        fill_momentum_table(state, n_iter2, beta_tab);
    }
    for (int i = threadIdx.x; i < NSET * MAXW * NV * 16; i += blockDim.x) red[i] = 0.0;
    const double inv_lw = 1.0 / state->l_w;
    const double m_scale_v = -inv_lw * 0x1p-52;
    const double m_scale = __hiloint2double(__builtin_amdgcn_readfirstlane(__double2hiint(m_scale_v)),
                                            __builtin_amdgcn_readfirstlane(__double2loint(m_scale_v)));

    const int m16 = lane & 15, q = lane >> 4;
    const int sw_row = (m16 >= 4 && m16 < 12) ? 1 : 0;
    const int qs = q ^ sw_row;
    const int c_row = 8 * (q & 1) + 4 * (q >> 1);
    const int mC = m16 ^ ((q == 1 || q == 2) ? 4 : 0);
    const int e_col = wcol0 + 4 * (m16 & 3) + (m16 >> 2);
    const int k_col = wcol0 + 4 * q;
    double a1r[4][NKC > 0 ? NKC : 1];
    double a2r[4][4];
    v4i pdg[7];
    int pj = 0, pl = 0;
    while ((pl + 1) * (pl + 2) / 2 <= m16) ++pl;
    pj = m16 - pl * (pl + 1) / 2;
    {
        const bool pair_ok = m16 < NP;
        const bool a2_ok = (m16 & 3) < NU;
#pragma unroll
        for (int t = 0; t < 4; ++t) {
#pragma unroll
            for (int kc = 0; kc < NKC; ++kc) {
                const int row = kc * 4 + q, col = e_col + 16 * t;
                a1r[t][kc] = (row < n_c && col < S) ? -alpha[(int64_t)row * S + col] : 0.0;
            }
#pragma unroll
            for (int r = 0; r < 4; ++r) {
                const int col = k_col + 16 * t + r;
                a2r[t][r] = (col < S && a2_ok) ? alpha[(int64_t)(n_c + (m16 & 3)) * S + col] * inv_lw : 0.0;
            }
        }
#pragma unroll
        for (int g = 0; g < 4; ++g) {
            unsigned int lo[4], hi[4], tl[4], th[4];
#pragma unroll
            for (int i = 0; i < 4; ++i) {
                const int col = wcol0 + 16 * q + 4 * g + i;
                const bool in = pair_ok && col < S;
                const double aj = in ? alpha[(int64_t)(n_c + pj) * S + col] : 0.0;
                const double al = in ? alpha[(int64_t)(n_c + pl) * S + col] : 0.0;
                z_to_biased(aj, al, lo[i], hi[i]);
            }
            transpose4(lo, tl);
            transpose4(hi, th);
            pdg[0][g] = (int)(tl[0] ^ 0x80808080u);
            pdg[1][g] = (int)(tl[1] ^ 0x80808080u);
            pdg[2][g] = (int)(tl[2] ^ 0x80808080u);
            pdg[3][g] = (int)(tl[3] ^ 0x80808080u);
            pdg[4][g] = (int)(th[0] ^ 0x80808080u);
            pdg[5][g] = (int)(th[1] ^ 0x80808080u);
            pdg[6][g] = (int)th[2];
        }
    }
    __syncthreads();

    double bu[4] = {0.0, 0.0, 0.0, 0.0};
    double u2_acc = 0.0;
    DMF2_STAMP_DECL
    const int64_t nblk = (N + 15) / 16;
    const int nk = (int)((nblk - blockIdx.x + gridDim.x - 1) / gridDim.x);

    const int ld_row = lane >> 5;
    const int ld_col = (lane & 31) * 2;
    int ld_gcol = wcol0 + ld_col;
    const int last_pair = (S - 1) & ~1;
    if (ld_gcol > last_pair) ld_gcol = last_pair;
    const int d_row = lane >> 3, d_col = (lane & 7) * 8;
    const int ld_col_sw = ((lane & 31) ^ 2) * 2;
    v2d pv[NSET][XS ? 1 : 8];
    v4u pd[NSET][2], px[NSET][XS ? 2 : 1];
    double nrt[NSET][NKC > 0 ? NKC : 1];
    double pu, pup;
    constexpr int RPWB = 64 / NU;
    const int rl = lane / NU, jb = lane - rl * NU;
    const bool b_lane = rl < 16 && rl < RPWB;
    const unsigned int v_off = (unsigned int)(ld_row * S + ld_gcol) * 8u;
    const unsigned int d_off = (unsigned int)(d_row * SD + wcol0 + d_col) * 2u;
    const unsigned int r_off = (unsigned int)(m16 * NCT + q) * 8u;
    const unsigned int u_off = b_lane ? (unsigned int)lane * 8u : 0xFFFFFFF0u;
    auto span = [](int64_t bytes) { return (unsigned int)(bytes < 0 ? 0 : (bytes > 0x7FFFFFFF ? 0x7FFFFFFF : bytes)); };
    auto prefetch_u = [&](int64_t blk) {
        const int64_t r0 = blk * 16;
        const int64_t left = N - r0;
        const __amdgpu_buffer_rsrc_t ru = __builtin_amdgcn_make_buffer_rsrc((void*)(u + r0 * NU), 0, span(left * NU * 8), 0x00020000);
        const __amdgpu_buffer_rsrc_t rp = __builtin_amdgcn_make_buffer_rsrc((void*)(u_prev + r0 * NU), 0, span(left * NU * 8), 0x00020000);
        const v2u a = __builtin_amdgcn_raw_buffer_load_b64(ru, u_off, 0, 0);
        const v2u b = __builtin_amdgcn_raw_buffer_load_b64(rp, u_off, 0, 0);
        pu = __hiloint2double((int)a.y, (int)a.x);
        pup = __hiloint2double((int)b.y, (int)b.x);
    };
    auto prefetch_tile = [&](int64_t blk, int set) {
        const int64_t r0 = blk * 16;
        const int64_t left = N - r0;
        if (NKC > 0) {
            const __amdgpu_buffer_rsrc_t rr = __builtin_amdgcn_make_buffer_rsrc((void*)(Rtp + r0 * NCT), 0, span(left * NCT * 8), 0x00020000);
#pragma unroll
            for (int kc = 0; kc < NKC; ++kc) {
                const v2u a = __builtin_amdgcn_raw_buffer_load_b64(rr, r_off, kc * 32, 0);
                nrt[set][kc] = __hiloint2double((int)a.y, (int)a.x);
            }
        }
        if constexpr (!XS) {
            const __amdgpu_buffer_rsrc_t rv = __builtin_amdgcn_make_buffer_rsrc((void*)(V + r0 * S), 0, span(left * S * 8), 0x00020000);
#pragma unroll
            for (int i = 0; i < 8; ++i) {
                const v4u a = __builtin_amdgcn_raw_buffer_load_b128(rv, v_off, 2 * i * S * 8, 0);
                pv[set][i] = v2d{__hiloint2double((int)a.y, (int)a.x), __hiloint2double((int)a.w, (int)a.z)};
            }
        } else {
            const __amdgpu_buffer_rsrc_t rx = __builtin_amdgcn_make_buffer_rsrc((void*)(X16 + r0 * SD), 0, span((int64_t)16 * SD * 2), 0x00020000);
            px[set][0] = __builtin_amdgcn_raw_buffer_load_b128(rx, d_off, 0, 0);
            px[set][1] = __builtin_amdgcn_raw_buffer_load_b128(rx, d_off, 8 * SD * 2, 0);
        }
        {
            const __amdgpu_buffer_rsrc_t rd = __builtin_amdgcn_make_buffer_rsrc((void*)(D16 + r0 * SD), 0, span((int64_t)16 * SD * 2), 0x00020000);
            pd[set][0] = __builtin_amdgcn_raw_buffer_load_b128(rd, d_off, 0, 0);
            pd[set][1] = __builtin_amdgcn_raw_buffer_load_b128(rd, d_off, 8 * SD * 2, 0);
        }
    };
    auto pair_set = [&](int s) { return (PAIR && s + 1 < nk && wave == (s + 1) % NW) ? 1 : 0; };
    if (nk > 0) {
        prefetch_u(blockIdx.x + (int64_t)pair_set(0) * gridDim.x);
        prefetch_tile(blockIdx.x, 0);
        if (PAIR && nk > 1) prefetch_tile(blockIdx.x + gridDim.x, 1);
    }

    double* __restrict__ const mine_c = red + (size_t)wave * NV * 16 + (m16 * NU + q) * SLOT;
    double* __restrict__ const mine_m1 = red + (size_t)wave * NV * 16 + (4 * q * NU + pl) * SLOT + 1 + (pj - pl + NU) % NU;
    double* __restrict__ const mine_m2 = red + (size_t)wave * NV * 16 + (4 * q * NU + pj) * SLOT + 1 + (pl - pj) % NU;

    auto tile_store = [&](int set, int rslot) {
        const BlockTile T = block_tile(set);
        if constexpr (DEFER_C) {
#pragma unroll
            for (int i = 0; i < 2; ++i)
                *reinterpret_cast<v2u*>(ring_at(rslot, 8 * i + d_row, 2 * (lane & 7))) =
                    v2u{__builtin_amdgcn_perm(px[set][i].y, px[set][i].x, 0x06040200u),
                        __builtin_amdgcn_perm(px[set][i].w, px[set][i].z, 0x06040200u)};
        } else if constexpr (XS) {
#pragma unroll
            for (int i = 0; i < 2; ++i) *reinterpret_cast<v4u*>(T.X + (8 * i + d_row) * kRowD + d_col) = px[set][i];
        } else {
#pragma unroll
            for (int i = 0; i < 8; ++i)
                *reinterpret_cast<v2d*>(T.V + (2 * i + ld_row) * kRowV + ((i >= 2 && i < 6) ? ld_col_sw : ld_col)) = pv[set][i];
        }
#ifndef DMF_ABLATE_DSTORE
#pragma unroll
        for (int i = 0; i < 2; ++i) *reinterpret_cast<v4u*>(T.D + (8 * i + d_row) * kRowD + d_col) = pd[set][i];
#endif
    };

    auto phase_a = [&](int set, int rslot, int st_a, int st_p) {
        const BlockTile T = block_tile(set);
        const double* __restrict__ const tileV = T.V;
        unsigned short* __restrict__ const tileD = T.D;
        unsigned short* __restrict__ const tileX = T.X;
        const double (&rtop)[NKC > 0 ? NKC : 1] = nrt[set];
        struct StripV {
            v2d v01, v23;
            v2u dw;
        };
        struct StripX {
            v2u dw, xw;
        };
        using Strip = std::conditional_t<XS, StripX, StripV>;
        auto load_strip = [&](int t, Strip& R) {
            if constexpr (DEFER_C) {
                R.xw.x = *ring_at(rslot, m16, 4 * t + q);
            } else if constexpr (XS) {
                R.xw = *reinterpret_cast<const v2u*>(tileX + m16 * kRowD + t * 16 + 4 * q);
            } else {
                const double* __restrict__ tv = tileV + m16 * kRowV + t * 16 + 4 * qs;
                R.v01 = *reinterpret_cast<const v2d*>(tv);
                R.v23 = *reinterpret_cast<const v2d*>(tv + 2);
            }
            R.dw = *reinterpret_cast<const v2u*>(tileD + m16 * kRowD + t * 16 + 4 * q);
        };
        double csm0 = 0.0, csm1 = 0.0;
        auto e_init = [&](const Strip& R) {
            if constexpr (XS) return v4d{0.0, 0.0, 0.0, 0.0};
            else return v4d{R.v01.x, R.v01.y, R.v23.x, R.v23.y};
        };
        auto run_strip = [&](const Strip& R, v4d e, const Strip& Rn, const double (&a1n)[NKC > 0 ? NKC : 1],
                             const double (&a2)[4], bool has_next) {
            const v4d d = {(double)(R.dw.x & 0xFFFFu), (double)(R.dw.x >> 16), (double)(R.dw.y & 0xFFFFu), (double)(R.dw.y >> 16)};
            v4d w;
            if constexpr (XS) {
                const v4d x = DEFER_C ? v4d{(double)(R.xw.x & 0xFFu), (double)((R.xw.x >> 8) & 0xFFu), (double)((R.xw.x >> 16) & 0xFFu), (double)(R.xw.x >> 24)}
                                      : v4d{(double)(R.xw.x & 0xFFFFu), (double)(R.xw.x >> 16), (double)(R.xw.y & 0xFFFFu), (double)(R.xw.y >> 16)};
#pragma unroll
                for (int r = 0; r < 4; ++r) w[r] = fma(d[r], e[r], x[r]);
            } else {
                w = d * e;
            }
            v4d en = e_init(Rn);
#pragma unroll
            for (int r = 0; r < 4; ++r) {
                if (r & 1) csm1 = __builtin_amdgcn_mfma_f64_4x4x4f64(a2[r], w[r], csm1, 0, 0, 0);
                else csm0 = __builtin_amdgcn_mfma_f64_4x4x4f64(a2[r], w[r], csm0, 0, 0, 0);
                if (has_next && r < NKC) en = __builtin_amdgcn_mfma_f64_16x16x4f64(a1n[r], rtop[r], en, 0, 0, 0);
            }
            return en;
        };
#ifdef DMF_ABLATE_E
        const double csm = XS ? (double)tileX[m16 * kRowD + 4 * q] : tileV[m16 * kRowV + 4 * qs];
#else
        Strip sa, sb;
        load_strip(0, sa);
        load_strip(1, sb);
        __builtin_amdgcn_sched_barrier(0);
        v4d e0 = e_init(sa);
#pragma unroll
        for (int kc = 0; kc < NKC; ++kc) e0 = __builtin_amdgcn_mfma_f64_16x16x4f64(a1r[0][kc], rtop[kc], e0, 0, 0, 0);
        const v4d e1 = run_strip(sa, e0, sb, a1r[1], a2r[0], true);
        load_strip(2, sa);
        __builtin_amdgcn_sched_barrier(0);
        const v4d e2 = run_strip(sb, e1, sa, a1r[2], a2r[1], true);
        load_strip(3, sb);
        __builtin_amdgcn_sched_barrier(0);
        const v4d e3 = run_strip(sa, e2, sb, a1r[3], a2r[2], true);
        (void)run_strip(sb, e3, sb, a1r[3], a2r[3], false);
        const double csm = csm0 + csm1;
#endif
        v4i mw[8];
#pragma unroll
        for (int w8 = 0; w8 < 8; ++w8) mw[w8] = v4i{0, 0, 0, 0};
#ifndef DMF_ABLATE_M
        {
            const v4u wa = *reinterpret_cast<const v4u*>(tileD + m16 * kRowD + 16 * q);
            const v4u wb = *reinterpret_cast<const v4u*>(tileD + m16 * kRowD + 16 * q + 8);
            const unsigned int e0 = wa.x + 0x00800080u, e1 = wa.y + 0x00800080u, e2 = wa.z + 0x00800080u, e3 = wa.w + 0x00800080u;
            const unsigned int e4 = wb.x + 0x00800080u, e5 = wb.y + 0x00800080u, e6 = wb.z + 0x00800080u, e7 = wb.w + 0x00800080u;
            const v4i c0 = {(int)(__builtin_amdgcn_perm(e1, e0, 0x06040200u) ^ 0x80808080u),
                            (int)(__builtin_amdgcn_perm(e3, e2, 0x06040200u) ^ 0x80808080u),
                            (int)(__builtin_amdgcn_perm(e5, e4, 0x06040200u) ^ 0x80808080u),
                            (int)(__builtin_amdgcn_perm(e7, e6, 0x06040200u) ^ 0x80808080u)};
#pragma unroll
            for (int t = 0; t < 7; ++t) mw[t] = __builtin_amdgcn_mfma_i32_16x16x64_i8(c0, pdg[t], mw[t], 0, 0, 0);
            if (nd == 2) {
                const v4i c1 = {(int)__builtin_amdgcn_perm(e1, e0, 0x07050301u), (int)__builtin_amdgcn_perm(e3, e2, 0x07050301u),
                                (int)__builtin_amdgcn_perm(e5, e4, 0x07050301u), (int)__builtin_amdgcn_perm(e7, e6, 0x07050301u)};
#pragma unroll
                for (int t = 0; t < 7; ++t) mw[t + 1] = __builtin_amdgcn_mfma_i32_16x16x64_i8(c1, pdg[t], mw[t + 1], 0, 0, 0);
            }
        }
#endif
        double mrow[4];
#ifdef DMF_ABLATE_M
#pragma unroll
        for (int rr = 0; rr < 4; ++rr) mrow[rr] = 0.25 * (rr == (m16 & 3));
#else
#pragma unroll
        for (int rr = 0; rr < 4; ++rr) {
#ifndef DMF_CHAIN_NO_I32
            const double lo = fma((double)(mw[3][rr] * 256 + mw[2][rr]), 65536.0, (double)(mw[1][rr] * 256 + mw[0][rr]));
            const double hi = fma((double)(mw[7][rr] * 256 + mw[6][rr]), 65536.0, (double)(mw[5][rr] * 256 + mw[4][rr]));
#else
            const double lo = fma(fma(fma((double)mw[3][rr], 256.0, (double)mw[2][rr]), 256.0, (double)mw[1][rr]), 256.0, (double)mw[0][rr]);
            const double hi = fma(fma(fma((double)mw[7][rr], 256.0, (double)mw[6][rr]), 256.0, (double)mw[5][rr]), 256.0, (double)mw[4][rr]);
#endif
            mrow[rr] = fma(hi, 0x1p32, lo) * m_scale;
        }
#endif
        DMF2_STAMP(st_a)
        {
            const size_t so = (size_t)set * MAXW * NV * 16;
            if (q < NU) mine_c[so] = csm;
            if (m16 < NP) {
#pragma unroll
                for (int rr = 0; rr < 4; ++rr) mine_m1[so + rr * NU * SLOT] = mrow[rr];
                if (pj != pl) {
#pragma unroll
                    for (int rr = 0; rr < 4; ++rr) mine_m2[so + rr * NU * SLOT] = mrow[rr];
                }
            }
        }
        DMF2_STAMP(st_p)
    };

    auto phase_b = [&](int uset, int set, int64_t row0, double uu0, double up0) {
        __builtin_amdgcn_s_setprio(3);
        DMF2_SUB_BEGIN
        const bool ok = b_lane && row0 + rl < N;
        const int lane0 = lane - jb;
        const int rlc = rl < 16 ? rl : 15;
        double cj = 0.0, Ms[NU];
#pragma unroll
        for (int l = 0; l < NU; ++l) Ms[l] = 0.0;
        {
            const double* __restrict__ slot = red + (size_t)set * MAXW * NV * 16 + (rlc * NU + jb) * SLOT;
#pragma unroll 1
            for (int w0 = 0; w0 < MAXW; w0 += 4) {
                v2d part[4][SLOT / 2];
#pragma unroll
                for (int w = 0; w < 4; ++w)
#pragma unroll
                    for (int h = 0; h < SLOT / 2; ++h)
                        part[w][h] = *reinterpret_cast<const v2d*>(slot + (w0 + w) * NV * 16 + 2 * h);
#pragma unroll
                for (int w = 0; w < 4; ++w) {
                    cj += part[w][0].x;
#pragma unroll
                    for (int l = 0; l < NU; ++l) Ms[l] += (l & 1) ? part[w][(l + 1) / 2].x : part[w][l / 2].y;
                }
            }
        }
        double uu = uu0, up = up0;
        DMF2_SUB(8)
#ifndef DMF_CHAIN_NO_UNROLL
        if (XS && MAXW == 4 && n_iter2 == kUnrolledSteps) {
            const double bvec = beta_tab[lane < kUnrolledSteps ? lane : kUnrolledSteps - 1];
// ... 91 lines not shown
        const int bset = pair_set(s);
        const bool my_turn = bset == 1 || wave == s % NW;
        const double uu0 = pu;
        const double up0 = pup;
        __builtin_amdgcn_wave_barrier();
        __builtin_amdgcn_s_setprio(0);
        DMF2_STAMP(0)
        phase_a(0, rs0, 1, 2);
        if (has2) phase_a(1, rs0 + 1, 11, 12);
        asm volatile("s_waitcnt lgkmcnt(0)" ::: "memory");
        __builtin_amdgcn_s_barrier();
        DMF2_STAMP(3)
#ifndef DMF_V2_NO_STAGGER
        if constexpr (!DEFER_C) {
            if (!my_turn) __builtin_amdgcn_s_sleep(DMF_V2_STAGGER);
        } else if (DMF_V2_STAGGER_DEFER > 0) {
            if (!b_role) __builtin_amdgcn_s_sleep(DMF_V2_STAGGER_DEFER);
        }
#endif
        if (s + NSET < nk) {
            const int64_t nb = blk + NSET * (int64_t)gridDim.x;
            prefetch_u(nb + (int64_t)pair_set(s + NSET) * gridDim.x);
            prefetch_tile(nb, 0);
            if (PAIR && s + 3 < nk) prefetch_tile(nb + gridDim.x, 1);
        }
        if (b_role) { DMF2_STAMP(7) } else { DMF2_STAMP(16) }
        if (my_turn) phase_b((DEFER_C ? rs0 : 0) + bset, bset, (blk + (int64_t)bset * gridDim.x) * 16, uu0, up0);
        DMF2_STAMP(4)
        if constexpr (DEFER_C) {
            if (!b_role) {
                if (DMF_V2_DEFER_PRIO > 0) __builtin_amdgcn_s_setprio(DMF_V2_DEFER_PRIO);
#pragma unroll 1
                for (int pp = cyc < 2 ? 0 : cyc - 2; pp < cyc; ++pp) {
                    phase_c_ring(pp, 0);
                    phase_c_ring(pp, 1);
                }
                if (DMF_V2_DEFER_PRIO > 0) __builtin_amdgcn_s_setprio(0);
            }
            DMF2_STAMP(6)
        }
        asm volatile("s_waitcnt lgkmcnt(0)" ::: "memory");
        __builtin_amdgcn_s_barrier();
        if (b_role) { DMF2_STAMP(5) } else { DMF2_STAMP(17) }
        if constexpr (!DEFER_C) {
            phase_c(0);
            DMF2_STAMP(6)
            if (has2) phase_c(1);
            __builtin_amdgcn_s_setprio(0);
            DMF2_STAMP(13)
        }
    }
    if constexpr (DEFER_C) {
        if (nk > 0) {
            const int last = (nk - 1) >> 1;
            const bool lone = (nk & 1) != 0;
            const int first = ((wave >> 1) != (last & 1) || last == 0) ? last : last - 1;
#pragma unroll 1
            for (int pp = first; pp <= last; ++pp) {
                phase_c_ring(pp, 0);
                if (pp < last || !lone) phase_c_ring(pp, 1);
            }
        }
        DMF2_STAMP(13)
    }

    DMF2_STAMP_FLUSH
    const double w2 = wave_sum(u2_acc);
    if (lane == 0) u2red[wave] = w2;
    __syncthreads();
    if (q < NU) {
#pragma unroll
        for (int t = 0; t < 4; ++t) {
            const int sC = wcol0 + (DEFER_C ? 4 * m16 + t : 16 * t + m16);
            if (sC < S) slab[((int64_t)blockIdx.x * NU + q) * S + sC] = bu[t];
        }
    }
    if (threadIdx.x == 0) {
        double tot = 0.0;
        for (int w = 0; w < NW; ++w) tot += u2red[w];
        u2_partials[blockIdx.x] = tot;
    }
}

size_t rowpass_v2_lds_bytes(int S, int n_u, int n_iter2, bool x16, bool pair = false, bool defer_c = false) {
    const int NW = (S + 63) / 64;
    const int maxw = NW <= 4 ? 4 : 8;
    const int nset = pair ? 2 : 1;
    const int nub = defer_c ? kDeferUbufSets : nset;
    const int nv = n_u * ((n_u + 2) & ~1);
    const size_t doubles = (size_t)((n_iter2 + 1) & ~1) + (size_t)nub * 16 * n_u + (size_t)nset * maxw * nv * 16 + maxw;
    const int tile = defer_c ? kTileDBytes2 : (x16 ? kTileBytesX : kTileBytes2);
    return doubles * sizeof(double) + (size_t)nset * NW * tile + (defer_c ? (size_t)NW * kRingBytes : 0);
}

bool rowpass_v2_supported(int S, int n_c, int n_u, int n_iter2) {
    if (S < 2 || S > 512 || n_c > 16 || n_u < 1 || n_u > 4) return false;
    return rowpass_v2_lds_bytes(S, n_u, n_iter2, false) <= (size_t)(S <= 256 ? 80 : 160) * 1024;
}

static int rowpass_v2_per_cu(int NW) {
    return per_cu_knob("DMF_V2_PER_CU", NW > 4 ? 1 : 8 / NW);
}

bool rowpass_v2_pair_fits(int S, int n_u, int n_iter2) {
    const int NW = (S + 63) / 64;
    if (NW < 2 || NW > 4) return false;
    return rowpass_v2_lds_bytes(S, n_u, n_iter2, true, true) * (size_t)rowpass_v2_per_cu(NW) <= (size_t)160 * 1024;
}

constexpr bool rowpass_v2_defer_instance(int nkc, int nu) { return !(nkc == 4 && nu >= 3); }
bool rowpass_v2_defer_fits(int S, int n_c, int n_u, int n_iter2) {
    const int NW = (S + 63) / 64;
    if (NW != 4 || !rowpass_v2_pair_fits(S, n_u, n_iter2) || !rowpass_v2_defer_instance((n_c + 3) / 4, n_u)) return false;
    const size_t lds = (rowpass_v2_lds_bytes(S, n_u, n_iter2, true, true, true) + 2047) & ~(size_t)2047;
    return lds * (size_t)rowpass_v2_per_cu(NW) <= (size_t)160 * 1024;
}

int rowpass_v2_grid(int64_t N, int S) {
    const int per_cu = rowpass_v2_per_cu((S + 63) / 64);
    const int64_t nblk = (N + 15) / 16;
    const int64_t g = 256 * per_cu;
    return (int)(nblk < g ? nblk : g);
}

hipError_t launch_rowpass_v2(const ProblemView& p, const IterateView& it, int n_iter2, const UScratch& scratch, int* grid_out,
                             bool pair, bool* paired_out, bool defer_c, bool* deferred_out, hipStream_t st) {
    const int S = p.S, NW = (S + 63) / 64;
    pair = pair && p.X16 != nullptr && rowpass_v2_pair_fits(S, it.n_u, n_iter2);
    if (paired_out != nullptr) *paired_out = pair;
    defer_c = defer_c && pair && rowpass_v2_defer_fits(S, p.n_c, it.n_u, n_iter2);
    if (deferred_out != nullptr) *deferred_out = defer_c;
    return dispatch_int<0, 4>((p.n_c + 3) / 4, [&](auto nkc) {
        return dispatch_bool(p.X16 != nullptr, [&](auto xs) {
            return dispatch_int<1, 4>(it.n_u, [&](auto nu) {
                const auto launch = [&](auto maxw, auto pair_t, auto defer_t) {
                    constexpr int NU = decltype(nu)::value, MAXW = decltype(maxw)::value;
                    constexpr bool XS = decltype(xs)::value, PAIR = decltype(pair_t)::value, DEFER_C = decltype(defer_t)::value;
                    constexpr auto kernel = k_rowpass_v2<decltype(nkc)::value, NU, MAXW, XS, PAIR, DEFER_C>;
                    const size_t lds = rowpass_v2_lds_bytes(S, NU, n_iter2, XS, PAIR, DEFER_C);
                    constexpr size_t kLdsCap = (size_t)(MAXW == 4 ? 80 : 160) * 1024;
                    if (NW > MAXW || (MAXW == 8 && NW <= 4) || (PAIR && NW < 2) || (DEFER_C && NW != 4) || lds > kLdsCap || p.N < 1 ||
                        p.SD < NW * 64 || (p.SD & 7) != 0 || p.ND < 1 || p.ND > 2)
                        return hipErrorInvalidValue;
                    if (lds > 48 * 1024) {
                        const hipError_t e = raise_dynamic_lds<kernel>(kLdsCap);
                        if (e != hipSuccess) return e;
                    }
                    const int grid = rowpass_v2_grid(p.N, S);
                    *grid_out = grid;
                    hipLaunchKernelGGL(kernel, dim3(grid), dim3(NW * 64), lds, st, p.V, p.D16, p.X16, p.SD, p.Rtp, it.alpha,
                                       it.u, it.u_prev, it.state, p.N, S, p.n_c, n_iter2, it.mode, p.ND, scratch.slab,
                                       scratch.u2_partials
#ifdef DMF_STAMPS
                                       , (unsigned long long*)nullptr
#endif
                                       );
                    return hipGetLastError();
                };
                if (S > 256) return launch(std::integral_constant<int, 8>{}, std::false_type{}, std::false_type{});
                if constexpr (decltype(xs)::value) {
                    if constexpr (rowpass_v2_defer_instance(decltype(nkc)::value, decltype(nu)::value)) {
                        if (pair && defer_c) return launch(std::integral_constant<int, 4>{}, std::true_type{}, std::true_type{});
                    }
                    if (pair) return launch(std::integral_constant<int, 4>{}, std::true_type{}, std::false_type{});
                }
                return launch(std::integral_constant<int, 4>{}, std::false_type{}, std::false_type{});
            });
        });
    });
}

}
```

demethify_amd/csrc/dmf_select.h:

```cpp
#pragma once
#include <cstddef>
#include <cstdint>

namespace dmf {

constexpr int kSplitInnerSteps = 50;
constexpr int kCmI8MinNu = 5;
constexpr int kSplitMinNu = 7;
constexpr int kGramI8MinFp64Acc = 48;
constexpr int kGramI8MinPairsNoKnown = 33;

struct ShapeKey {
    int64_t N = 0;
    int S = 0, n_c = 0, n_u = 0;
    int nd = 0;
    int SD = 0;
    bool x16 = false;
    bool rowpass_pair = true;
    bool rowpass_defer_c = true;
    bool x_byte = false;
    int level = 0;
    bool d_f32_exact = false;
    bool rtp_present = true;
    unsigned v_align = 0;
    unsigned rtp_align = 0;
    bool alpha_unit = true;
};

struct PathSpec {
    int u_path = 2;
    bool use_gram_spec = false, use_gram_mfma = false, use_u_big = false;
    bool use_v2 = false, use_cm_i8 = false, use_gram_i8 = false, use_fused = false;
    bool supported = true;
};

enum class RowKind {
    RowpassV2,
    CmI8InnerBu,
    CmI8InnerRows,
    RowpassFused,
    UPhaseBig,
    UPhaseMfmaSplit,
    UPhaseMfma,
    UPhaseGram,
    UStepDirect
};
enum class GramKind { InRowPass, I8, BuColsI8, GramU, GramMfma, Gram };
enum class AlphaKind { FrankWolfeRow16, FrankWolfe, PhaseRow16, PhaseLanes, Phase, PhaseDyn };

struct IterationPlan {
    RowKind row = RowKind::UStepDirect;
    GramKind gram = GramKind::Gram;
    AlphaKind alpha = AlphaKind::PhaseDyn;
};

PathSpec select_path(const ShapeKey& k);
IterationPlan plan_iteration(const ShapeKey& k, const PathSpec& s, int n_iter2, bool purity);
int describe_plan(const ShapeKey& k, const IterationPlan& plan, char* buf, size_t cap);
PathSpec standalone_spec(PathSpec s);
int describe_u_phase(const ShapeKey& k, const PathSpec& s, int n_iter2, bool purity, bool standalone, char* buf, size_t cap);

struct CostKey {
    int S = 0, n_c = 0, n_u = 0;
    bool d16 = false;
    int SD = 0;
    unsigned v_align = 0;
    bool rtp_present = true;
    int level = 0;
};
enum class CostKind {
    Cols,
    Cols2,
    Cols2Wide,
    Generic
};
struct CostPlan {
    CostKind kind = CostKind::Generic;
    int nkc = 0, nu = 0;
    bool d16 = false;
    bool odd = false;
    bool alpha_in_lds = false;
};
constexpr int kCostPartials = 1024;
CostPlan cost_plan(const CostKey& k);
int describe_cost_plan(const CostPlan& plan, char* buf, size_t cap);

}
```

demethify_amd/device.py:

```python
from __future__ import annotations

import ctypes as C
import os

import numpy as np

from . import _lib as L

_contexts: dict[int, "Context"] = {}


def _is_torch(x) -> bool:
    return type(x).__module__.startswith("torch")


def _host_f64(x, name):
    a = np.ascontiguousarray(x, dtype=np.float64)
    if not np.all(np.isfinite(a)):
        raise ValueError(f"{name} holds non-finite values (use --fillna)")
    return a


def _ptr(a):
    if a is None:
        return None
    if _is_torch(a) or hasattr(a, "data_ptr"):
        return C.c_void_p(a.data_ptr())
    return a.ctypes.data_as(C.c_void_p)


def pack_mask(mask) -> np.ndarray:
    m = np.asarray(mask)
    if m.ndim != 2:
        raise ValueError(f"a mask is N x S, got shape {m.shape}")
    return np.packbits(m.astype(bool, copy=False), axis=1, bitorder="little")


def mask_threshold(fraction) -> int:
    import math

    f = float(fraction)
    if not f > 0.0:
        return 0
    if f >= 1.0:
        return 1 << 53
    return math.ceil(f * 9007199254740992.0)


class Context:

    def __init__(self, device: int = 0, stream: int | None = None):
        self._lib = L.load()
        h = C.c_void_p()
        L.check(self._lib.dmf_context_create(int(device), C.c_void_p(stream) if stream else None, C.byref(h)),
                "dmf_context_create")
        self._h = h
        self.device = int(device)
        self.generic_level = 0

    def close(self):
        if getattr(self, "_h", None):
            self._lib.dmf_context_destroy(self._h)
            self._h = None

    def __del__(self):
        try:
            self.close()
        except Exception:
            pass

    def synchronize(self):
        L.check(self._lib.dmf_context_synchronize(self._h), "dmf_context_synchronize")

    def set_profiling(self, enabled, families=None):
        mode = int(bool(enabled))
        if mode and families is not None:
            mode = sum(1 << (1 + int(f)) for f in families)
        L.check(self._lib.dmf_context_set_profiling(self._h, mode), "dmf_context_set_profiling")

    def set_generic(self, level: int):
        L.check(self._lib.dmf_context_set_generic(self._h, int(level)), "dmf_context_set_generic")
        self.generic_level = int(level)

    def set_x16(self, enabled: bool):
        L.check(self._lib.dmf_context_set_x16(self._h, int(bool(enabled))), "dmf_context_set_x16")

    def set_rowpass_pair(self, enabled: bool):
        L.check(self._lib.dmf_context_set_rowpass_pair(self._h, int(bool(enabled))), "dmf_context_set_rowpass_pair")

    def set_rowpass_defer_c(self, enabled: bool):
        L.check(self._lib.dmf_context_set_rowpass_defer_c(self._h, int(bool(enabled))), "dmf_context_set_rowpass_defer_c")

    def set_stop_confirmation(self, mode: int):
        L.check(self._lib.dmf_context_set_stop_confirmation(self._h, int(mode)), "dmf_context_set_stop_confirmation")

    def reset_kernel_time(self):
        L.check(self._lib.dmf_context_reset_kernel_time(self._h), "dmf_context_reset_kernel_time")

    def kernel_time(self, family: int):
        ms, n = C.c_double(), C.c_int64()
        L.check(self._lib.dmf_context_kernel_time(self._h, int(family), C.byref(ms), C.byref(n)),
                "dmf_context_kernel_time")
        return ms.value, n.value

    def project_simplex(self, X, z=1.0):
        X = np.ascontiguousarray(X, dtype=np.float64)
        out = np.empty_like(X)
        K, S = X.shape
        L.check(self._lib.dmf_project_simplex(self._h, _ptr(X), K, S, float(z), 0, _ptr(out)),
                "dmf_project_simplex")
        return out

    def nnls_normal(self, G, mom):
        mom = np.ascontiguousarray(mom, dtype=np.float64)
        if mom.ndim != 2 or mom.shape[0] < 4 or mom.shape[0] % 2:
            raise ValueError(f"mom is (2 K + 2) x S, got shape {mom.shape}")
        K, S = mom.shape[0] // 2 - 1, mom.shape[1]
        G = np.asarray(G, dtype=np.float64)
        if G.shape == (S, K, K):
            if not np.array_equal(G, G.transpose(0, 2, 1)):
                raise ValueError("G must be symmetric")
            i, j = np.triu_indices(K)
            gb = np.empty((K * (K + 1) // 2, S), dtype=np.float64)
            gb[j * (j + 1) // 2 + i] = G[:, i, j].T
        elif G.shape == (K * (K + 1) // 2, S):
            gb = np.ascontiguousarray(G)
        else:
            raise ValueError(f"G shape {G.shape} is neither {(S, K, K)} nor {(K * (K + 1) // 2, S)}")
        out = np.full((K, S), np.nan, dtype=np.float64)
        status = np.full(S, -1, dtype=np.intc)
        L.check(self._lib.dmf_nnls_normal(self._h, _ptr(gb), _ptr(mom), K, S, _ptr(out),
                                          status.ctypes.data_as(C.POINTER(C.c_int))), "dmf_nnls_normal")
        return out, status

    def percentile_axis0(self, x, q):
        return self._percentile_axis0(x, q, "dmf_percentile_axis0")

    def nanpercentile_axis0(self, x, q):
        return self._percentile_axis0(x, q, "dmf_nanpercentile_axis0")

    def _percentile_axis0(self, x, q, entry):
        fn = getattr(self._lib, entry)
        qs = np.ascontiguousarray(np.atleast_1d(q), dtype=np.float64)
        if _is_torch(x) and x.is_cuda:
            import torch

            if x.dtype != torch.float64:
                raise TypeError(f"{entry[4:]} takes float64 data")
            x = x.contiguous()
            n, tail = x.shape[0], tuple(x.shape[1:])
            m = int(np.prod(tail, dtype=np.int64))
            out = torch.empty((len(qs),) + tail, dtype=torch.float64, device=x.device)
            torch.cuda.current_stream(x.device).synchronize()
            L.check(fn(self._h, _ptr(x), n, m, _ptr(qs), len(qs), L.DMF_PTR_DEVICE, _ptr(out)), entry)
            return out
        if _is_torch(x):
            x = x.numpy()
        x = np.ascontiguousarray(x, dtype=np.float64)
        n, tail = x.shape[0], tuple(x.shape[1:])
        m = int(np.prod(tail, dtype=np.int64))
        out = np.empty((len(qs),) + tail, dtype=np.float64)
        L.check(fn(self._h, _ptr(x), n, m, _ptr(qs), len(qs), 0, _ptr(out)), entry)
        return out


def get_context(device: int | None = None) -> Context:
    if device is None:
        device = int(os.environ.get("DEMETHIFY_DEVICE", os.environ.get("LOCAL_RANK", "0")))
    ctx = _contexts.get(device)
    if ctx is None:
        ctx = _contexts[device] = Context(device)
    return ctx


# ... 107 lines not shown
            if m.dtype == np.bool_:
                if m.shape != (self.N, self.S):
                    raise ValueError(f"mask shape {m.shape} != problem shape {(self.N, self.S)}")
                bits = pack_mask(m)
            elif m.dtype == np.uint8:
                if m.shape != (self.N, nb):
                    raise ValueError(f"packed mask shape {m.shape} != {(self.N, nb)} (ceil(S / 8) bytes per row)")
                bits = np.ascontiguousarray(m)
            else:
                raise TypeError("train_mask must be a bool N x S array or packed uint8 bits")
        h = C.c_void_p()
        L.check(self._lib.dmf_problem_mask(self.ctx._h, self._h, _ptr(bits), flags, C.byref(h)), "dmf_problem_mask")
        out = Problem._from_handle(self.ctx, h, self.N, self.S, self.n_c)
        out._keep = (self,)
        return out

    def close(self):
        if getattr(self, "_h", None):
            if getattr(self.ctx, "_h", None):
                self._lib.dmf_problem_destroy(self._h)
            self._h = None
            self._keep = ()

    def __del__(self):
        try:
            self.close()
        except Exception:
            pass

    def __enter__(self):
        return self

    def __exit__(self, *exc):
        self.close()

    def cost(self, u, alpha) -> float:
        alpha = np.ascontiguousarray(alpha, dtype=np.float64)
        n_u = 0
        if u is not None:
            u = np.ascontiguousarray(u, dtype=np.float64).reshape(self.N, -1)
            n_u = u.shape[1]
        if alpha.shape != (self.n_c + n_u, self.S):
            raise ValueError(f"alpha shape {alpha.shape} != {(self.n_c + n_u, self.S)}")
        out = C.c_double()
        L.check(self._lib.dmf_cost(self.ctx._h, self._h, _ptr(u) if n_u else None, n_u, _ptr(alpha), 0,
                                   C.byref(out)), "dmf_cost")
        return out.value

    def cost_describe(self, n_u: int) -> str:
        buf = C.create_string_buffer(128)
        L.check(self._lib.dmf_problem_cost_describe(self.ctx._h, self._h, int(n_u), buf, len(buf)),
                "dmf_problem_cost_describe")
        return buf.value.decode()

    def gram_known(self):
        out = np.empty(((self.n_c + 1) * (self.n_c + 2) // 2, self.S), dtype=np.float64)
        buf = C.create_string_buffer(256)
        L.check(self._lib.dmf_problem_gram_known(self._h, _ptr(out), buf, len(buf)), "dmf_problem_gram_known")
        return out, buf.value.decode()

    def report(self) -> dict:
        ints = (C.c_int64 * len(L.REPORT_INTS))()
        dbls = (C.c_double * len(L.REPORT_DBLS))()
        L.check(self._lib.dmf_problem_report(self._h, ints, dbls), "dmf_problem_report")
        out = {k: int(v) for k, v in zip(L.REPORT_INTS, ints)}
        out.update({k: float(v) for k, v in zip(L.REPORT_DBLS, dbls)})
        return out

    def copy_out(self, name: str, report: dict | None = None) -> np.ndarray:
        r = self.report() if report is None else report
        shape, dtype = {
            "V": ((r["N"], r["S"]), np.float64), "D": ((r["N"], r["S"]), np.float64),
            "Rt": ((r["N"], r["n_c"]), np.float64), "Rtp": ((r["N"], r["rtp_width"]), np.float64),
            "D16": ((r["N16"], r["SD"]), np.uint16), "X16": ((r["N16"], r["SD"]), np.uint16),
            "W16": ((r["N16"], r["SD"]), np.uint16),
            "Dt8": ((r["ND"], (r["N"] + 31) // 32, r["SD"] // 32, 32, 32), np.int8),
            "mask_bits": ((r["N"], (r["S"] + 7) // 8), np.uint8), "consts": ((6,), np.float64),
        }[name]
        out = np.empty(shape, dtype=dtype)
        L.check(self._lib.dmf_problem_copy_out(self._h, L.PROBLEM_ARRAYS[name], _ptr(out), out.nbytes),
                "dmf_problem_copy_out")
        return out

    def wls_intercept(self, u=None, target="v", host_arrays=None, f64_arrays=False):
        tg, u, n_u, flags = self._wls_args(u, target, f64_arrays)
        K = self.n_c + n_u
        out = np.zeros((K, self.S), dtype=np.float64)
        status = np.full(self.S, -1, dtype=np.intc)
        L.check(self._lib.dmf_wls_intercept(self.ctx._h, self._h, _ptr(u) if n_u else None, n_u, tg, flags, _ptr(out),
                                            status.ctypes.data_as(C.POINTER(C.c_int))), "dmf_wls_intercept")
        self.wls_status = status
        if (status == 2).any():
            raise ZeroDivisionError("Weights sum to zero, can't be normalized")
        redo = np.flatnonzero(status != 0)
        if redo.size:
            if host_arrays is None:
                raise RuntimeError(f"wls_intercept: the device did not solve samples {redo.tolist()} (rank-deficient "
                                   "profiles or iteration cap) and no host_arrays were given to solve them on the host")
            from .init_func import wls_intercept as host_wls

            meth_f, counts, R_full = host_arrays() if callable(host_arrays) else host_arrays
            for k in redo:
                x = counts[:, k:k + 1] * meth_f[:, k:k + 1] if target == "dv" else meth_f[:, k:k + 1]
                out[:, k:k + 1] = host_wls(x, counts[:, k:k + 1], R_full)
        return out

    def wls_moments(self, u=None, target="v", f64_arrays=False):
        tg, u, n_u, flags = self._wls_args(u, target, f64_arrays)
        out = np.empty((2 * (self.n_c + n_u) + 2, self.S), dtype=np.float64)
        L.check(self._lib.dmf_wls_moments(self.ctx._h, self._h, _ptr(u) if n_u else None, n_u, tg, flags, _ptr(out)),
                "dmf_wls_moments")
        return out

    def _wls_args(self, u, target, f64_arrays):
        try:
            tg = {"v": L.DMF_WLS_TARGET_V, "dv": L.DMF_WLS_TARGET_DV}[target]
        except KeyError:
            raise ValueError(f'target must be "v" or "dv", got {target!r}') from None
        flags, n_u = 0, 0
        if u is not None:
            if getattr(u, "is_cuda", False):
                from .staging import DeviceArray

                if isinstance(u, DeviceArray):
                    ok = u.ctx is self.ctx
                else:
                    ok = (_is_torch(u) and u.is_contiguous() and u.element_size() == 8 and u.is_floating_point()
                          and u.device.index == self.ctx.device)
                    if ok:
                        import torch

                        torch.cuda.current_stream(u.device).synchronize()
                if not ok:
                    raise ValueError("a device u must be a float64 staging.DeviceArray / contiguous CUDA tensor on the "
                                     "context's GPU")
                u = u.reshape(self.N, -1)
                flags = L.DMF_PTR_DEVICE
            else:
                u = _host_f64(u, "u").reshape(self.N, -1)
            n_u = int(u.shape[1])
        if f64_arrays:
            flags |= L.DMF_WLS_F64_ARRAYS
        return tg, u, n_u, flags

    def svd_gram(self, H1=None):
        if self.n_c:
            H1 = _host_f64(H1, "H1")
            if H1.shape != (self.n_c, self.S):
                raise ValueError(f"H1 shape {H1.shape} != {(self.n_c, self.S)}")
        else:
            H1 = None
        out = np.empty((self.S, self.S), dtype=np.float64)
        counts = (C.c_int64 * 2)()
        L.check(self._lib.dmf_svd_gram(self.ctx._h, self._h, _ptr(H1), 0, _ptr(out), counts), "dmf_svd_gram")
        return out, int(counts[0]), int(counts[1])

    def nndsvd(self, rank, keep_on_device=False, host_arrays=None):
        from .init_func import constrained_nndsvd, nndsvd_from_eig, nndsvd_initialize

        rank = int(rank)
        if rank < 1:
            raise ValueError(f"rank must be at least 1, got {rank}")

        def host_route():
            if host_arrays is None:
                raise RuntimeError("nndsvd: the device route does not take this problem and no host_arrays were given")
# ... 178 lines not shown
        it, conv = C.c_int64(), C.c_int()
        L.check(self._lib.dmf_solver_step(self._h, int(n_outer), int(n_iter2), float(tol), C.byref(it),
                                          C.byref(conv)), "dmf_solver_step")
        return it.value, bool(conv.value)

    def get(self):
        u = np.empty((self.problem.N, self.n_u), dtype=np.float64)
        alpha = np.empty((self.K, self.problem.S), dtype=np.float64)
        cost, it = C.c_double(), C.c_int64()
        L.check(self._lib.dmf_solver_get(self._h, 0, _ptr(u), _ptr(alpha), C.byref(cost), C.byref(it)),
                "dmf_solver_get")
        return u, alpha, cost.value, it.value

    def direct_cost(self) -> float:
        out = C.c_double()
        L.check(self._lib.dmf_solver_cost(self._h, C.byref(out)), "dmf_solver_cost")
        return out.value

    def holdout_error(self, full: Problem):
        ss, n = C.c_double(), C.c_int64()
        L.check(self._lib.dmf_solver_holdout_error(self._h, full._h, C.byref(ss), C.byref(n)), "dmf_solver_holdout_error")
        return ss.value, n.value

    def cost_begin(self):
        L.check(self._lib.dmf_solver_cost_begin(self._h), "dmf_solver_cost_begin")

    def cost_end(self) -> float:
        out = C.c_double()
        L.check(self._lib.dmf_solver_cost_end(self._h, C.byref(out)), "dmf_solver_cost_end")
        return out.value

    def describe(self, n_iter2: int = 20) -> str:
        buf = C.create_string_buffer(512)
        L.check(self._lib.dmf_solver_describe(self._h, int(n_iter2), buf, len(buf)), "dmf_solver_describe")
        return buf.value.decode()

    def u_phase_describe(self, n_iter2: int = 20, route="solver") -> str:
        buf = C.create_string_buffer(2048)
        L.check(self._lib.dmf_solver_u_phase_describe(self._h, int(n_iter2), _route(route), buf, len(buf)),
                "dmf_solver_u_phase_describe")
        return buf.value.decode()

    def gram(self, kind="integer"):
        try:
            k = {"integer": L.DMF_GRAM_INTEGER, "fp64": L.DMF_GRAM_FP64, "last": L.DMF_GRAM_LAST}[kind]
        except KeyError:
            raise ValueError(f'kind must be "integer", "fp64" or "last", got {kind!r}') from None
        out = np.empty(((self.K + 1) * (self.K + 2) // 2, self.problem.S), dtype=np.float64)
        buf = C.create_string_buffer(256)
        L.check(self._lib.dmf_solver_gram(self._h, k, _ptr(out), buf, len(buf)), "dmf_solver_gram")
        return out, buf.value.decode()

    def row_moments(self):
        n_u = self.n_u
        out = np.empty((self.problem.N, n_u + n_u * (n_u + 1) // 2), dtype=np.float64)
        buf = C.create_string_buffer(2048)
        L.check(self._lib.dmf_solver_row_moments(self._h, _ptr(out), buf, len(buf)), "dmf_solver_row_moments")
        return out, buf.value.decode()

    def momentum_state(self, arrays=True):
        sc = (C.c_double * len(L.MOMENTUM_SCALARS))()
        alpha_prev = np.empty((self.K, self.problem.S), dtype=np.float64) if arrays else None
        u_prev = np.empty((self.problem.N, self.n_u), dtype=np.float64) if arrays else None
        L.check(self._lib.dmf_solver_momentum_state(self._h, sc, _ptr(alpha_prev), _ptr(u_prev)),
                "dmf_solver_momentum_state")
        out = {name: (int(v) if i >= 11 else float(v)) for i, (name, v) in enumerate(zip(L.MOMENTUM_SCALARS, sc))}
        if arrays:
            out["alpha_prev"], out["u_prev"] = alpha_prev, u_prev
        return out

    def stop_info(self):
        on, nc, nu, cs = C.c_int(), C.c_int64(), C.c_int64(), C.c_double()
        L.check(self._lib.dmf_solver_stop_info(self._h, C.byref(on), C.byref(nc), C.byref(nu), C.byref(cs)),
                "dmf_solver_stop_info")
        return {"confirm_stops": bool(on.value), "n_confirmed": nc.value, "n_unconfirmed": nu.value,
                "last_stream_cost": cs.value}

    def rowpass_launches(self):
        total, paired = C.c_int64(), C.c_int64()
        L.check(self._lib.dmf_solver_rowpass_launches(self._h, C.byref(total), C.byref(paired)),
                "dmf_solver_rowpass_launches")
        return total.value, paired.value

    def rowpass_schedule_counts(self):
        total, paired, deferred = C.c_int64(), C.c_int64(), C.c_int64()
        L.check(self._lib.dmf_solver_rowpass_schedule_counts(self._h, C.byref(total), C.byref(paired), C.byref(deferred)),
                "dmf_solver_rowpass_schedule_counts")
        return total.value, paired.value, deferred.value

    def get_alpha(self):
        alpha = np.empty((self.K, self.problem.S), dtype=np.float64)
        L.check(self._lib.dmf_solver_get(self._h, 0, None, _ptr(alpha), None, None), "dmf_solver_get")
        return alpha

    def _on_device(self, t, floating):
        from .staging import DeviceArray

        ctx = self.problem.ctx
        if isinstance(t, DeviceArray):
            return t.ctx is ctx
        ok = (_is_torch(t) and t.is_cuda and t.is_contiguous() and t.element_size() == 8
              and t.is_floating_point() == floating and t.device.index == ctx.device)
        if ok:
            import torch

            ok = floating or t.dtype == torch.int64
        if ok:
            torch.cuda.current_stream(t.device).synchronize()
        return ok

    def match_components(self, anchor, idx=None):
        on_device = self._on_device
        if not on_device(anchor, True):
            raise ValueError("anchor must be a float64 staging.DeviceArray / contiguous CUDA tensor on the context's GPU")
        n_el = int(np.prod(tuple(anchor.shape)))
        if n_el == 0 or n_el % self.n_u:
            raise ValueError(f"anchor shape {tuple(anchor.shape)} does not hold rows of {self.n_u} profiles")
        n_rows = n_el // self.n_u
        if idx is not None:
            if not on_device(idx, False):
                raise ValueError("idx must be the int64 row indices in HBM (staging.indices_to_device) on the context's GPU")
            if int(np.prod(tuple(idx.shape))) != self.problem.N:
                raise ValueError(f"idx holds {int(np.prod(tuple(idx.shape)))} indices, the problem has {self.problem.N} rows")
        P = np.empty((self.n_u, self.n_u), dtype=np.float64)
        L.check(self._lib.dmf_solver_match_components(self._h, _ptr(anchor), n_rows, _ptr(idx), _ptr(P)),
                "dmf_solver_match_components")
        return P

    def copy_u_to(self, tensor, columns=None):
        if not (_is_torch(tensor) and tensor.is_cuda and tensor.is_contiguous() and tensor.numel() == self.problem.N * self.n_u
                and tensor.element_size() == 8 and tensor.device.index == self.problem.ctx.device):
            raise ValueError("copy_u_to needs a contiguous float64 CUDA tensor of N * n_u elements on the context's GPU")
        if columns is not None:
            cols = np.ascontiguousarray(columns, dtype=np.int32).ravel()
            if cols.size != self.n_u or not np.array_equal(np.sort(cols), np.arange(self.n_u)):
                raise ValueError(f"columns must be a permutation of 0..{self.n_u - 1}, got {list(np.ravel(columns))}")
            L.check(self._lib.dmf_solver_get_u_permuted(self._h, cols.ctypes.data_as(C.POINTER(C.c_int32)), _ptr(tensor)),
                    "dmf_solver_get_u_permuted")
            return
        L.check(self._lib.dmf_solver_get(self._h, L.DMF_PTR_DEVICE, _ptr(tensor), None, None, None), "dmf_solver_get")

    def copy_u_by_cpg(self, tensor, idx, n_rows, columns=None):
        n_rows = int(n_rows)
        if not (_is_torch(tensor) and tensor.is_cuda and tensor.is_contiguous() and tensor.numel() == n_rows * self.n_u
                and n_rows >= 1 and tensor.element_size() == 8 and tensor.is_floating_point()
                and tensor.device.index == self.problem.ctx.device):
            raise ValueError("copy_u_by_cpg needs a contiguous float64 CUDA tensor of n_rows * n_u elements on the context's GPU")
        if not self._on_device(idx, False):
            raise ValueError("idx must be the int64 row indices in HBM (staging.indices_to_device) on the context's GPU")
        if int(np.prod(tuple(idx.shape))) != self.problem.N:
            raise ValueError(f"idx holds {int(np.prod(tuple(idx.shape)))} indices, the problem has {self.problem.N} rows")
        cols = None
        if columns is not None:
            cols = np.ascontiguousarray(columns, dtype=np.int32).ravel()
            if cols.size != self.n_u or not np.array_equal(np.sort(cols), np.arange(self.n_u)):
                raise ValueError(f"columns must be a permutation of 0..{self.n_u - 1}, got {list(np.ravel(columns))}")
            cols = cols.ctypes.data_as(C.POINTER(C.c_int32))
        L.check(self._lib.dmf_solver_get_u_by_row(self._h, _ptr(idx), n_rows, cols, _ptr(tensor)), "dmf_solver_get_u_by_row")

    def get_cost(self):
        cost, it = C.c_double(), C.c_int64()
        L.check(self._lib.dmf_solver_get(self._h, 0, None, None, C.byref(cost), C.byref(it)), "dmf_solver_get")
        return cost.value, it.value

    def close(self):
        if getattr(self, "_h", None):
# ... 15 lines not shown
```

include/demethify_hip.h:

```cpp
#ifndef DEMETHIFY_HIP_H
#define DEMETHIFY_HIP_H

#include <stddef.h>
#include <stdint.h>

#ifdef __cplusplus
extern "C" {
#endif

typedef enum dmf_status {
    DMF_OK = 0,
    DMF_ERR_BAD_ARG = 1,
    DMF_ERR_BAD_SHAPE = 2,
    DMF_ERR_HIP = 3,
    DMF_ERR_NONFINITE = 4,
    DMF_ERR_UNSUPPORTED = 5,
    DMF_ERR_NO_DEVICE = 6
} dmf_status;

enum {
    DMF_PTR_DEVICE = 1,
    DMF_COUNTS_F64 = 2,
    DMF_INIT_IN_UNIT_RANGE = 4
};

enum {
    DMF_SELECT_COUNTS_F32_EXACT = 1,
    DMF_SELECT_PURITY = 2,
    DMF_SELECT_ALPHA_OUTSIDE_UNIT = 4,
    DMF_SELECT_V_UNALIGNED = 8,
    DMF_SELECT_X16 = 16
};

enum {
    DMF_MODE_PARTIAL = 0,
    DMF_MODE_UNSUPERVISED = 1
};

enum {
    DMF_KERNEL_ROWPASS = 0,
    DMF_KERNEL_GRAM = 1,
    DMF_KERNEL_ALPHA = 2,
    DMF_KERNEL_COST = 3,
    DMF_KERNEL_FAMILIES = 4
};

typedef struct dmf_context dmf_context;
typedef struct dmf_problem dmf_problem;
typedef struct dmf_solver dmf_solver;

const char* dmf_status_string(int status);
const char* dmf_last_error(void);
int dmf_abi_version(void);

int dmf_context_create(int device, void* stream, dmf_context** out);
int dmf_context_destroy(dmf_context* ctx);
int dmf_context_synchronize(dmf_context* ctx);
int dmf_context_set_profiling(dmf_context* ctx, int enabled);
int dmf_context_kernel_time(dmf_context* ctx, int family, double* total_ms, int64_t* launches);
int dmf_context_reset_kernel_time(dmf_context* ctx);
int dmf_context_set_generic(dmf_context* ctx, int level);
int dmf_context_set_x16(dmf_context* ctx, int enabled);
int dmf_context_set_rowpass_pair(dmf_context* ctx, int enabled);
int dmf_context_set_rowpass_defer_c(dmf_context* ctx, int enabled);
int dmf_context_set_stop_confirmation(dmf_context* ctx, int mode);

int dmf_problem_create(dmf_context* ctx, int64_t N, int64_t S, int64_t n_c,
                       const double* V, const void* counts, const double* Rt,
                       int flags, dmf_problem** out);
int dmf_problem_gather(dmf_context* ctx, const dmf_problem* src, const int64_t* idx,
                       int64_t n_idx, dmf_problem** out);
int dmf_problem_gather_device(dmf_context* ctx, const dmf_problem* src, const int64_t* idx_dev,
                              int64_t n_idx, dmf_problem** out);
int dmf_problem_mask(dmf_context* ctx, const dmf_problem* src, const uint8_t* train_bits, int flags, dmf_problem** out);
int dmf_problem_destroy(dmf_problem* p);
int dmf_problem_shape(const dmf_problem* p, int64_t* N, int64_t* S, int64_t* n_c);
int dmf_problem_gram_known(const dmf_problem* p, double* out, char* out_text, int64_t cap);
enum { DMF_REPORT_INTS = 16, DMF_REPORT_DBLS = 8 };
int dmf_problem_report(const dmf_problem* p, int64_t* out_ints, double* out_dbls);
enum {
    DMF_ARRAY_V = 0, DMF_ARRAY_D = 1, DMF_ARRAY_RT = 2, DMF_ARRAY_RTP = 3, DMF_ARRAY_D16 = 4, DMF_ARRAY_X16 = 5,
    DMF_ARRAY_W16 = 6, DMF_ARRAY_DT8 = 7, DMF_ARRAY_MASK_BITS = 8, DMF_ARRAY_CONSTS = 9
};
int dmf_problem_copy_out(const dmf_problem* p, int which, void* out, int64_t bytes);

int dmf_cost(dmf_context* ctx, const dmf_problem* p, const double* u, int64_t n_u,
             const double* alpha, int flags, double* out_cost);
int dmf_cost_describe(int64_t S, int64_t n_c, int64_t n_u, int has_u16, int64_t SD, int v_align, int rtp_present, int level,
                      char* buf, int64_t cap);
int dmf_problem_cost_describe(dmf_context* ctx, const dmf_problem* p, int64_t n_u, char* buf, int64_t cap);
int dmf_gram_i8_describe(int64_t N, int64_t S, int64_t n_c, int64_t n_u, int nd, char* buf, int64_t cap);
int dmf_project_simplex(dmf_context* ctx, const double* X, int64_t K, int64_t S, double z,
                        int flags, double* out);
int dmf_update_u(dmf_context* ctx, const dmf_problem* p, const double* u, const double* u_prev,
                 const double* alpha, int64_t n_u, int64_t n_iter2, int mode, int flags,
                 double* scalars_io, double* out_u, double* out_u_prev);
int dmf_update_alpha(dmf_context* ctx, const dmf_problem* p, const double* u, int64_t n_u,
                     const double* alpha, const double* alpha_prev, int64_t n_iter2, int flags,
                     double* scalars_io, double* out_alpha, double* out_alpha_prev);

enum { DMF_WLS_TARGET_V = 0, DMF_WLS_TARGET_DV = 1 };
enum { DMF_WLS_F64_ARRAYS = 8 };
int dmf_wls_intercept(dmf_context* ctx, const dmf_problem* p, const double* u, int64_t n_u, int target,
                      int flags, double* out_alpha, int* out_status);
int dmf_wls_moments(dmf_context* ctx, const dmf_problem* p, const double* u, int64_t n_u, int target, int flags,
                    double* out_mom);
int dmf_nnls_normal(dmf_context* ctx, const double* gb, const double* mom, int64_t K, int64_t S, double* out_alpha,
                    int* out_status);

int dmf_svd_gram(dmf_context* ctx, const dmf_problem* p, const double* H1, int flags, double* out_C, int64_t* out_flags);
int dmf_svd_factor(dmf_context* ctx, const dmf_problem* p, const double* H1, const double* E_over_sigma, int64_t rank,
                   int flags, double* out_norms, void** out_T);
int dmf_svd_finish(dmf_context* ctx, void* T, int64_t N, int64_t rank, const double* sign, const double* scale, int flags,
                   double* out_u);

int dmf_percentile_axis0(dmf_context* ctx, const double* x, int64_t n, int64_t m, const double* q,
                         int64_t n_q, int flags, double* out);
int dmf_nanpercentile_axis0(dmf_context* ctx, const double* x, int64_t n, int64_t m, const double* q,
                            int64_t n_q, int flags, double* out);

int dmf_solver_create(dmf_context* ctx, const dmf_problem* p, const double* u0,
                      const double* alpha0, int64_t n_u, int mode, int flags, dmf_solver** out);
int dmf_solver_set_purity(dmf_solver* s, const double* purity, int flags);
int dmf_solver_step(dmf_solver* s, int64_t n_outer, int64_t n_iter2, double tol,
                    int64_t* iters_done_total, int* converged);
int dmf_solver_get(dmf_solver* s, int flags, double* out_u, double* out_alpha,
                   double* out_cost, int64_t* out_iters);
int dmf_solver_match_components(dmf_solver* s, const void* anchor_dev, int64_t n_anchor_rows, const int64_t* idx_dev,
                                double* out_P);
int dmf_solver_get_u_permuted(dmf_solver* s, const int32_t* src_col, void* dst_dev);
int dmf_solver_get_u_by_row(dmf_solver* s, const int64_t* idx_dev, int64_t n_dst_rows, const int32_t* src_col ,
                            void* dst_dev);
int dmf_solver_cost(dmf_solver* s, double* out_cost);
int dmf_solver_cost_begin(dmf_solver* s);
int dmf_solver_cost_end(dmf_solver* s, double* out_cost);
int dmf_solver_holdout_error(dmf_solver* s, const dmf_problem* full, double* sum_sq, int64_t* n_test);
enum { DMF_GRAM_INTEGER = 0, DMF_GRAM_FP64 = 1, DMF_GRAM_LAST = 2 };
int dmf_solver_gram(dmf_solver* s, int kind, double* out_gb, char* out_text, int64_t cap);
int dmf_solver_row_moments(dmf_solver* s, double* out_cm, char* out_text, int64_t cap);
enum { DMF_MOMENTUM_SCALARS = 16 };
int dmf_solver_momentum_state(const dmf_solver* s, double* scalars, double* alpha_prev, double* u_prev);
int dmf_solver_destroy(dmf_solver* s);
int dmf_solver_describe(const dmf_solver* s, int64_t n_iter2, char* buf, int64_t cap);
int dmf_select_describe(int64_t N, int64_t S, int64_t n_c, int64_t n_u, int nd, int level, int64_t n_iter2, int flags,
                        char* buf, int64_t cap);
enum { DMF_ROUTE_SOLVER = 0, DMF_ROUTE_UPDATE_U = 1 };
int dmf_u_phase_describe(int64_t N, int64_t S, int64_t n_c, int64_t n_u, int nd, int level, int64_t n_iter2, int flags, int route,
                         char* buf, int64_t cap);
int dmf_solver_u_phase_describe(const dmf_solver* s, int64_t n_iter2, int route, char* buf, int64_t cap);
int dmf_solver_stop_info(const dmf_solver* s, int* confirm_stops, int64_t* n_confirmed, int64_t* n_unconfirmed,
                         double* last_stream_cost);
int dmf_solver_rowpass_launches(const dmf_solver* s, int64_t* total, int64_t* paired);
int dmf_solver_rowpass_schedule_counts(const dmf_solver* s, int64_t* total, int64_t* paired, int64_t* deferred);
int dmf_solve(dmf_context* ctx, const dmf_problem* p, const double* u0, const double* alpha0,
              int64_t n_u, int mode, int64_t n_iter1, int64_t n_iter2, double tol, int flags,
              double* out_u, double* out_alpha, double* out_cost, int64_t* out_iters);

int dmf_solve_small_supported(int64_t N, int64_t S, int64_t n_c, int64_t n_u, int mode);
int dmf_solve_small(dmf_context* ctx, const dmf_problem* p, int64_t B, const int64_t* idx, const double* u0,
                    const double* alpha0, int64_t n_u, int mode, int64_t n_iter1, int64_t n_iter2, double tol,
                    int64_t iters_per_launch, int flags, double* out_u, double* out_alpha, double* out_cost,
                    int64_t* out_iters);
int dmf_solve_small_purity(dmf_context* ctx, const dmf_problem* p, int64_t B, const int64_t* idx, const double* u0,
                           const double* alpha0, const double* purity, int64_t n_u, int mode, int64_t n_iter1,
                           int64_t n_iter2, double tol, int64_t iters_per_launch, int flags, double* out_u,
                           double* out_alpha, double* out_cost, int64_t* out_iters);

int dmf_table_scan(const char* path, char sep, int64_t* n_rows, int* col_percent_modified, int* col_valid_coverage,
                   int* n_cols);
int dmf_table_read(const char* path, char sep, int col_percent_modified, int col_valid_coverage, int64_t n_rows,
                   double* out_freq, int64_t stride_freq, double divide_by, int64_t* out_cov, int64_t stride_cov,
                   int n_threads);
void* dmf_host_alloc(size_t bytes, int* pinned);
void dmf_host_free(void* p, int pinned);

int dmf_write_interval_csv(const char* path, const char* header_line, const double* lower, const double* upper,
                           int64_t n_rows, int n_cols, int numpy_scalar_repr, int n_threads);

int dmf_stage_upload(dmf_context* ctx, const void* host, size_t bytes, void** out_dev);
int dmf_stage_free(dmf_context* ctx, void* dev);
int dmf_stage_download(dmf_context* ctx, const void* dev, size_t bytes, void* host);

int dmf_mask_draw(dmf_context* ctx, uint32_t key[624], int* pos, int64_t N, int64_t S,
                  uint64_t threshold, void** out_bits, int64_t* n_kept);

#ifdef __cplusplus
}
#endif
#endif
```

Baseline: 1853 outer iters/s.

## Pre-pack X and D into 8-bit ring-layout byte images for rowpass

At problem creation, when counts fit in a byte and S is between 193 and 256, builds 8-bit images of X16 and D16 laid out in the LDS ring-slot swizzle order. The deferred-C paired rowpass then loads one 16-byte vector per lane for each of X and D instead of two 16-bit loads apiece, stores them straight into LDS, and unpacks bytes in place of halfwords. This is meant to halve the global traffic for the count matrices and to simplify the LDS staging, at the cost of extra device memory and a one-time build pass.

```diff
diff --git a/demethify_amd/_lib.py b/demethify_amd/_lib.py
--- a/demethify_amd/_lib.py
+++ b/demethify_amd/_lib.py
@@ -23,6 +23,7 @@
                "rtp_width", "rtp_borrows_rt", "n_test", "d_f32_exact")
 REPORT_DBLS = ("kDsq", "kRtSumsq", "kDmax", "kF32ResidualMax", "kIntCountMax", "kRtOutsideUnit", "x16_dev", "x16_sum")
 PROBLEM_ARRAYS = {"V": 0, "D": 1, "Rt": 2, "Rtp": 3, "D16": 4, "X16": 5, "W16": 6, "Dt8": 7, "mask_bits": 8, "consts": 9}
+PROBLEM_BYTE_IMAGES = {"X8": 10, "D8": 11}
 DMF_MODE_PARTIAL = 0
 DMF_MODE_UNSUPERVISED = 1
 MAX_K = 64
@@ -55,6 +56,10 @@
     "dmf_context_set_x16": (C.c_int, [_p, C.c_int]),
     "dmf_context_set_rowpass_pair": (C.c_int, [_p, C.c_int]),
     "dmf_context_set_rowpass_defer_c": (C.c_int, [_p, C.c_int]),
+    "dmf_context_set_rowpass_bytes": (C.c_int, [_p, C.c_int]),
+    "dmf_problem_has_byte_images": (C.c_int, [_p, C.POINTER(C.c_int)]),
+    "dmf_rowpass_image_offset": (C.c_int, [C.c_int, C.c_int]),
+    "dmf_solver_rowpass_byte_launches": (C.c_int, [_p, C.POINTER(_i64)]),
     "dmf_context_set_stop_confirmation": (C.c_int, [_p, C.c_int]),
     "dmf_problem_create": (C.c_int, [_p, _i64, _i64, _i64, _p, _p, _p, C.c_int, C.POINTER(_p)]),
     "dmf_problem_gather": (C.c_int, [_p, _p, _p, _i64, C.POINTER(_p)]),
diff --git a/demethify_amd/csrc/dmf_api.h b/demethify_amd/csrc/dmf_api.h
--- a/demethify_amd/csrc/dmf_api.h
+++ b/demethify_amd/csrc/dmf_api.h
@@ -14,6 +14,7 @@
 
 #include "../../include/demethify_hip.h"
 #include "dmf_internal.h"
+#include "dmf_rowpass_image.h"
 #include "dmf_select.h"
 
 using dmf::SolverState;
@@ -55,6 +56,7 @@
     bool x16 = true;
     bool rowpass_pair = true;
     bool rowpass_defer_c = true;
+    bool rowpass_bytes = true;
     double* scratch = nullptr;
     hipMemPool_t pool = nullptr;
     std::unordered_map<void*, size_t> live;
@@ -173,6 +175,7 @@
     int64_t N16 = 0, plane_stride = 0;
     dmf_api::DevBuf<unsigned short> X16;
     double x16_dev = 0.0, x16_sum = 0.0;
+    dmf_api::DevBuf<unsigned char> X8, D8;
     bool d_f32_exact = false;
     dmf_api::DevBuf<double> gb_known;
     dmf::GramRan known_ran;
@@ -182,6 +185,7 @@
     dmf::ProblemView view() const {
         dmf::ProblemView v;
         v.V = V, v.D = D, v.D16 = D16, v.X16 = X16, v.Dt8 = Dt8;
+        v.X8 = X8, v.D8 = D8;
         v.plane_stride = plane_stride, v.SD = SD, v.ND = ND;
         v.Rt = Rt, v.Rtp = Rtp;
         v.N = N, v.S = (int)S, v.n_c = (int)n_c;
@@ -228,6 +232,7 @@
     long long cf_stream_iter = -1;
     long long n_rowpass = 0, n_rowpass_pair = 0;
     long long n_rowpass_defer = 0;
+    long long n_rowpass_bytes = 0;
     long long n_confirmed = 0, n_unconfirmed = 0;
     dmf::IterateView iterate() const {
         dmf::IterateView it;
diff --git a/demethify_amd/csrc/dmf_api_context.hip b/demethify_amd/csrc/dmf_api_context.hip
--- a/demethify_amd/csrc/dmf_api_context.hip
+++ b/demethify_amd/csrc/dmf_api_context.hip
@@ -324,6 +324,12 @@
     return DMF_OK;
 }
 
+int dmf_context_set_rowpass_bytes(dmf_context* ctx, int enabled) {
+    if (ctx == nullptr || enabled < 0 || enabled > 1) return DMF_ERR_BAD_ARG;
+    ctx->rowpass_bytes = enabled != 0;
+    return DMF_OK;
+}
+
 int dmf_context_set_stop_confirmation(dmf_context* ctx, int mode) {
     if (ctx == nullptr || mode < 0 || mode > 2) return DMF_ERR_BAD_ARG;
     ctx->stop_confirmation = mode;
diff --git a/demethify_amd/csrc/dmf_api_problem.hip b/demethify_amd/csrc/dmf_api_problem.hip
--- a/demethify_amd/csrc/dmf_api_problem.hip
+++ b/demethify_amd/csrc/dmf_api_problem.hip
@@ -13,6 +13,16 @@
     HIP_TRY(p->Dt8.alloc(ctx, (size_t)p->plane_stride * ND));
     if (x16) HIP_TRY(p->X16.alloc(ctx, u16_elems));
     if (w16) HIP_TRY(p->W16.alloc(ctx, u16_elems));
+    return DMF_OK;
+}
+
+static int build_rowpass_images(dmf_problem* p) {
+    dmf_context* ctx = p->ctx;
+    if (p->X16 == nullptr || p->D16 == nullptr || !(p->h_consts[kIntCountMax] <= 255.0) || p->S < 193 || p->S > 256) return DMF_OK;
+    const size_t bytes = (size_t)p->N16 * p->SD;
+    HIP_TRY(p->X8.alloc(ctx, bytes));
+    HIP_TRY(p->D8.alloc(ctx, bytes));
+    HIP_TRY(dmf::launch_build_rowpass_images(p->X16, p->D16, p->N16, p->SD, p->X8, p->D8, ctx->stream));
     return DMF_OK;
 }
 
@@ -75,6 +85,8 @@
             }
         }
     }
+
+    DMF_TRY(build_rowpass_images(p));
 
     if (n_c > 0 && n_c <= 48) {
         const int nct = (int)((n_c + 3) / 4 * 4);
@@ -389,11 +401,24 @@
         case DMF_ARRAY_DT8: src = p->Dt8, size = (size_t)p->plane_stride * p->ND; break;
         case DMF_ARRAY_MASK_BITS: src = p->mask_bits, size = (size_t)p->N * (size_t)((p->S + 7) / 8); break;
         case DMF_ARRAY_CONSTS: src = p->consts, size = kProblemConsts * sizeof(double); break;
+        case DMF_ARRAY_X8: src = p->X8, size = (size_t)p->N16 * p->SD; break;
+        case DMF_ARRAY_D8: src = p->D8, size = (size_t)p->N16 * p->SD; break;
         default: return DMF_ERR_BAD_ARG;
     }
     if (src == nullptr || size == 0) return DMF_ERR_BAD_ARG;
     if (bytes < 0 || (size_t)bytes != size) return DMF_ERR_BAD_SHAPE;
     return export_array(ctx, src, size, 0, out);
+}
+
+int dmf_problem_has_byte_images(const dmf_problem* p, int* out) {
+    if (p == nullptr || out == nullptr) return DMF_ERR_BAD_ARG;
+    *out = p->X8 != nullptr && p->D8 != nullptr;
+    return DMF_OK;
+}
+
+int dmf_rowpass_image_offset(int row, int sample) {
+    if (row < 0 || row > 15 || sample < 0 || sample > 63) return -1;
+    return dmf::rowpass_image_byte(row, sample);
 }
 
 int dmf_problem_shape(const dmf_problem* p, int64_t* N, int64_t* S, int64_t* n_c) {
diff --git a/demethify_amd/csrc/dmf_api_solver.hip b/demethify_amd/csrc/dmf_api_solver.hip
--- a/demethify_amd/csrc/dmf_api_solver.hip
+++ b/demethify_amd/csrc/dmf_api_solver.hip
@@ -147,16 +147,18 @@
     const dmf::IterationPlan plan = dmf::plan_iteration(s->key, s->spec, n_iter2, s->purity != nullptr);
     if (plan.row == dmf::RowKind::RowpassV2) {
         int grid = 0;
-        bool paired = false, deferred = false;
+        bool paired = false, deferred = false, bytes = false;
         {
             FamilyScope scope(ctx, DMF_KERNEL_ROWPASS);
             dmf::ProblemView pv = p->view();
             if (!s->key.x16) pv.X16 = nullptr;
+            if (!s->key.rowpass_bytes) pv.X8 = nullptr, pv.D8 = nullptr;
             HIP_TRY(dmf::launch_rowpass_v2(pv, s->iterate(), n_iter2, s->scratch(), &grid, s->key.rowpass_pair, &paired,
-                                           s->key.rowpass_defer_c && s->key.x_byte, &deferred, ctx->stream));
+                                           s->key.rowpass_defer_c && s->key.x_byte, &deferred, &bytes, ctx->stream));
             ++s->n_rowpass;
             s->n_rowpass_pair += paired ? 1 : 0;
             s->n_rowpass_defer += deferred ? 1 : 0;
+            s->n_rowpass_bytes += bytes ? 1 : 0;
         }
         return enqueue_gram_i8_tail(s, plan.alpha, n_iter2, grid);
     }
@@ -291,6 +293,7 @@
     key.x16 = key.nd > 0 && p->X16 != nullptr;
     key.rowpass_pair = ctx->rowpass_pair;
     key.rowpass_defer_c = ctx->rowpass_defer_c;
+    key.rowpass_bytes = ctx->rowpass_bytes;
     key.x_byte = key.x16 && p->h_consts[kIntCountMax] <= 255.0;
     key.level = ctx->generic_level;
     key.d_f32_exact = p->d_f32_exact;
@@ -734,6 +737,12 @@
     return DMF_OK;
 }
 
+int dmf_solver_rowpass_byte_launches(const dmf_solver* s, int64_t* bytes) {
+    if (s == nullptr || bytes == nullptr) return DMF_ERR_BAD_ARG;
+    *bytes = s->n_rowpass_bytes;
+    return DMF_OK;
+}
+
 int dmf_solve(dmf_context* ctx, const dmf_problem* p, const double* u0, const double* alpha0, int64_t n_u,
               int mode, int64_t n_iter1, int64_t n_iter2, double tol, int flags, double* out_u,
               double* out_alpha, double* out_cost, int64_t* out_iters) {
diff --git a/demethify_amd/csrc/dmf_internal.h b/demethify_amd/csrc/dmf_internal.h
--- a/demethify_amd/csrc/dmf_internal.h
+++ b/demethify_amd/csrc/dmf_internal.h
@@ -58,6 +58,8 @@
     const double* D = nullptr;
     const unsigned short* D16 = nullptr;
     const unsigned short* X16 = nullptr;
+    const unsigned char* X8 = nullptr;
+    const unsigned char* D8 = nullptr;
     const signed char* Dt8 = nullptr;
     int64_t plane_stride = 0;
     int SD = 0, ND = 0;
@@ -286,7 +288,9 @@
 bool rowpass_v2_supported(int S, int n_c, int n_u, int n_iter2);
 int rowpass_v2_grid(int64_t N, int S);
 hipError_t launch_rowpass_v2(const ProblemView& p, const IterateView& it, int n_iter2, const UScratch& scratch, int* grid_out,
-                             bool pair, bool* paired_out, bool defer_c, bool* deferred_out, hipStream_t st);
+                             bool pair, bool* paired_out, bool defer_c, bool* deferred_out, bool* bytes_out, hipStream_t st);
+hipError_t launch_build_rowpass_images(const unsigned short* X16, const unsigned short* D16, int64_t N16, int SD,
+                                       unsigned char* X8, unsigned char* D8, hipStream_t st);
 bool rowpass_v2_pair_fits(int S, int n_u, int n_iter2);
 bool gram_i8_supported(int n_c, int n_u, int ND, int64_t N, int SD);
 struct GramI8Plan {
diff --git a/demethify_amd/csrc/dmf_kernels_rowpass2.hip b/demethify_amd/csrc/dmf_kernels_rowpass2.hip
--- a/demethify_amd/csrc/dmf_kernels_rowpass2.hip
+++ b/demethify_amd/csrc/dmf_kernels_rowpass2.hip
@@ -3,6 +3,7 @@
 #include "dmf_internal.h"
 #include "dmf_ustep.h"
 #include "dmf_fixedpoint.h"
+#include "dmf_rowpass_image.h"
 #include <cstdlib>
 #include <type_traits>
 
@@ -58,6 +59,7 @@
 constexpr int kRingBlockBytes = 16 * 64;
 constexpr int kRingBytes = 6 * kRingBlockBytes;
 constexpr int kDeferUbufSets = 6;
+constexpr int kTileDBytes8 = kRowpassImageBytes;
 }
 
 template <int NU, bool AT_PREV>
@@ -89,7 +91,7 @@
     }
 }
 
-template <int NKC, int NU, int MAXW = 4, bool XS = false, bool PAIR = false, bool DEFER_C = false>
+template <int NKC, int NU, int MAXW = 4, bool XS = false, bool PAIR = false, bool DEFER_C = false, bool BYTES = false>
 __global__ __launch_bounds__(64 * MAXW, MAXW == 4 ? 2 : 1) void k_rowpass_v2(
     const double* __restrict__ V, const unsigned short* __restrict__ D16, const unsigned short* __restrict__ X16, int SD,
     const double* __restrict__ Rtp,
@@ -103,6 +105,7 @@
     static_assert(NU >= 1 && NU <= 4, "one phase-B pass per block, 4x4x4 MFMA for the c product");
     static_assert(!PAIR || (XS && MAXW == 4), "the pair schedule: X16 form, two workgroups per CU");
     static_assert(!DEFER_C || PAIR, "the deferred-C schedule is a pair schedule");
+    static_assert(!BYTES || DEFER_C, "the byte images are the deferred-C schedule's");
     constexpr int NSET = PAIR ? 2 : 1;
     constexpr int NUB = DEFER_C ? kDeferUbufSets : NSET;
     constexpr int NCT = 4 * NKC;
@@ -121,7 +124,7 @@
     double* __restrict__ ubuf = beta_tab + ((n_iter2 + 1) & ~1);
     double* __restrict__ red = ubuf + NUB * 16 * NU;
     double* __restrict__ u2red = red + NSET * MAXW * NV * 16;
-    constexpr int TB = XS ? (DEFER_C ? kTileDBytes2 : kTileBytesX) : kTileBytes2;
+    constexpr int TB = XS ? (BYTES ? kTileDBytes8 : DEFER_C ? kTileDBytes2 : kTileBytesX) : kTileBytes2;
     char* __restrict__ tile = reinterpret_cast<char*>(u2red + MAXW) + (size_t)wave * TB;
     struct BlockTile {
         double* V;
@@ -136,6 +139,9 @@
     auto ring_at = [&](int slot, int row, int dword) {
         return ring + slot * (kRingBlockBytes / 4) + (4 * (row & 3) + (row >> 2)) * 16 + ((dword + 4 * (row & 3)) & 15);
     };
+    static_assert(rowpass_image_dword(7, 9) == (4 * 3 + 1) * 16 + ((9 + 12) & 15) && kRingBlockBytes == kRowpassImageBytes,
+                  "a ring slot is an image of dmf_rowpass_image.h");
+    auto dtile8 = [&](int set) { return reinterpret_cast<unsigned int*>(tile + (size_t)set * NW * TB); };
 
     if (const double* __restrict__ mrow = momentum_row(state, n_iter2)) {
         const double lw_prev = state->l_w_prev, lw = state->l_w;
@@ -217,14 +223,15 @@
     const int d_row = lane >> 3, d_col = (lane & 7) * 8;
     const int ld_col_sw = ((lane & 31) ^ 2) * 2;
     v2d pv[NSET][XS ? 1 : 8];
-    v4u pd[NSET][2], px[NSET][XS ? 2 : 1];
+    v4u pd[NSET][BYTES ? 1 : 2], px[NSET][BYTES ? 1 : XS ? 2 : 1];
     double nrt[NSET][NKC > 0 ? NKC : 1];
     double pu, pup;
     constexpr int RPWB = 64 / NU;
     const int rl = lane / NU, jb = lane - rl * NU;
     const bool b_lane = rl < 16 && rl < RPWB;
     const unsigned int v_off = (unsigned int)(ld_row * S + ld_gcol) * 8u;
-    const unsigned int d_off = (unsigned int)(d_row * SD + wcol0 + d_col) * 2u;
+    const unsigned int d_off = BYTES ? (unsigned int)(wave * kRowpassImageBytes + lane * 16)
+                                     : (unsigned int)(d_row * SD + wcol0 + d_col) * 2u;
     const unsigned int r_off = (unsigned int)(m16 * NCT + q) * 8u;
     const unsigned int u_off = b_lane ? (unsigned int)lane * 8u : 0xFFFFFFF0u;
     auto span = [](int64_t bytes) { return (unsigned int)(bytes < 0 ? 0 : (bytes > 0x7FFFFFFF ? 0x7FFFFFFF : bytes)); };
@@ -249,7 +256,14 @@
                 nrt[set][kc] = __hiloint2double((int)a.y, (int)a.x);
             }
         }
-        if constexpr (!XS) {
+        if constexpr (BYTES) {
+            const unsigned char* const X8 = reinterpret_cast<const unsigned char*>(X16);
+            const unsigned char* const D8 = reinterpret_cast<const unsigned char*>(D16);
+            const __amdgpu_buffer_rsrc_t rx = __builtin_amdgcn_make_buffer_rsrc((void*)(X8 + r0 * SD), 0, span((int64_t)16 * SD), 0x00020000);
+            const __amdgpu_buffer_rsrc_t rd = __builtin_amdgcn_make_buffer_rsrc((void*)(D8 + r0 * SD), 0, span((int64_t)16 * SD), 0x00020000);
+            px[set][0] = __builtin_amdgcn_raw_buffer_load_b128(rx, d_off, 0, 0);
+            pd[set][0] = __builtin_amdgcn_raw_buffer_load_b128(rd, d_off, 0, 0);
+        } else if constexpr (!XS) {
             const __amdgpu_buffer_rsrc_t rv = __builtin_amdgcn_make_buffer_rsrc((void*)(V + r0 * S), 0, span(left * S * 8), 0x00020000);
 #pragma unroll
             for (int i = 0; i < 8; ++i) {
@@ -261,7 +275,7 @@
             px[set][0] = __builtin_amdgcn_raw_buffer_load_b128(rx, d_off, 0, 0);
             px[set][1] = __builtin_amdgcn_raw_buffer_load_b128(rx, d_off, 8 * SD * 2, 0);
         }
-        {
+        if constexpr (!BYTES) {
             const __amdgpu_buffer_rsrc_t rd = __builtin_amdgcn_make_buffer_rsrc((void*)(D16 + r0 * SD), 0, span((int64_t)16 * SD * 2), 0x00020000);
             pd[set][0] = __builtin_amdgcn_raw_buffer_load_b128(rd, d_off, 0, 0);
             pd[set][1] = __builtin_amdgcn_raw_buffer_load_b128(rd, d_off, 8 * SD * 2, 0);
@@ -280,7 +294,12 @@
 
     auto tile_store = [&](int set, int rslot) {
         const BlockTile T = block_tile(set);
-        if constexpr (DEFER_C) {
+        if constexpr (BYTES) {
+            *reinterpret_cast<v4u*>(ring + rslot * (kRingBlockBytes / 4) + 4 * lane) = px[set][0];
+#ifndef DMF_ABLATE_DSTORE
+            *reinterpret_cast<v4u*>(dtile8(set) + 4 * lane) = pd[set][0];
+#endif
+        } else if constexpr (DEFER_C) {
 #pragma unroll
             for (int i = 0; i < 2; ++i)
                 *reinterpret_cast<v2u*>(ring_at(rslot, 8 * i + d_row, 2 * (lane & 7))) =
@@ -295,8 +314,10 @@
                 *reinterpret_cast<v2d*>(T.V + (2 * i + ld_row) * kRowV + ((i >= 2 && i < 6) ? ld_col_sw : ld_col)) = pv[set][i];
         }
 #ifndef DMF_ABLATE_DSTORE
-#pragma unroll
-        for (int i = 0; i < 2; ++i) *reinterpret_cast<v4u*>(T.D + (8 * i + d_row) * kRowD + d_col) = pd[set][i];
+        if constexpr (!BYTES) {
+#pragma unroll
+            for (int i = 0; i < 2; ++i) *reinterpret_cast<v4u*>(T.D + (8 * i + d_row) * kRowD + d_col) = pd[set][i];
+        }
 #endif
     };
 
@@ -324,7 +345,8 @@
                 R.v01 = *reinterpret_cast<const v2d*>(tv);
                 R.v23 = *reinterpret_cast<const v2d*>(tv + 2);
             }
-            R.dw = *reinterpret_cast<const v2u*>(tileD + m16 * kRowD + t * 16 + 4 * q);
+            if constexpr (BYTES) R.dw.x = dtile8(set)[rowpass_image_dword(m16, 4 * t + q)];
+            else R.dw = *reinterpret_cast<const v2u*>(tileD + m16 * kRowD + t * 16 + 4 * q);
         };
         double csm0 = 0.0, csm1 = 0.0;
         auto e_init = [&](const Strip& R) {
@@ -333,7 +355,8 @@
         };
         auto run_strip = [&](const Strip& R, v4d e, const Strip& Rn, const double (&a1n)[NKC > 0 ? NKC : 1],
                              const double (&a2)[4], bool has_next) {
-            const v4d d = {(double)(R.dw.x & 0xFFFFu), (double)(R.dw.x >> 16), (double)(R.dw.y & 0xFFFFu), (double)(R.dw.y >> 16)};
+            const v4d d = BYTES ? v4d{(double)(R.dw.x & 0xFFu), (double)((R.dw.x >> 8) & 0xFFu), (double)((R.dw.x >> 16) & 0xFFu), (double)(R.dw.x >> 24)}
+                                : v4d{(double)(R.dw.x & 0xFFFFu), (double)(R.dw.x >> 16), (double)(R.dw.y & 0xFFFFu), (double)(R.dw.y >> 16)};
             v4d w;
             if constexpr (XS) {
                 const v4d x = DEFER_C ? v4d{(double)(R.xw.x & 0xFFu), (double)((R.xw.x >> 8) & 0xFFu), (double)((R.xw.x >> 16) & 0xFFu), (double)(R.xw.x >> 24)}
@@ -376,7 +399,18 @@
 #pragma unroll
         for (int w8 = 0; w8 < 8; ++w8) mw[w8] = v4i{0, 0, 0, 0};
 #ifndef DMF_ABLATE_M
-        {
+        if constexpr (BYTES) {
+            const v4u wd = *reinterpret_cast<const v4u*>(dtile8(set) + rowpass_image_dword(m16, 4 * q));
+            const v4i c0 = {(int)wd.x, (int)wd.y, (int)wd.z, (int)wd.w};
+#pragma unroll
+            for (int t = 0; t < 7; ++t) mw[t] = __builtin_amdgcn_mfma_i32_16x16x64_i8(c0, pdg[t], mw[t], 0, 0, 0);
+            if (nd == 2) {
+                const v4i c1 = {(int)((wd.x >> 7) & 0x01010101u), (int)((wd.y >> 7) & 0x01010101u),
+                                (int)((wd.z >> 7) & 0x01010101u), (int)((wd.w >> 7) & 0x01010101u)};
+#pragma unroll
+                for (int t = 0; t < 7; ++t) mw[t + 1] = __builtin_amdgcn_mfma_i32_16x16x64_i8(c1, pdg[t], mw[t + 1], 0, 0, 0);
+            }
+        } else {
             const v4u wa = *reinterpret_cast<const v4u*>(tileD + m16 * kRowD + 16 * q);
             const v4u wb = *reinterpret_cast<const v4u*>(tileD + m16 * kRowD + 16 * q + 8);
             const unsigned int e0 = wa.x + 0x00800080u, e1 = wa.y + 0x00800080u, e2 = wa.z + 0x00800080u, e3 = wa.w + 0x00800080u;
@@ -634,14 +668,43 @@
     }
 }
 
-size_t rowpass_v2_lds_bytes(int S, int n_u, int n_iter2, bool x16, bool pair = false, bool defer_c = false) {
+__global__ __launch_bounds__(256) void k_build_rowpass_images(const unsigned short* __restrict__ X16, const unsigned short* __restrict__ D16,
+                                                              int SD, int64_t pieces, unsigned char* __restrict__ X8,
+                                                              unsigned char* __restrict__ D8) {
+    const int64_t i = (int64_t)blockIdx.x * blockDim.x + threadIdx.x;
+    if (i >= pieces) return;
+    const int l = (int)(i & 63), groups = SD >> 6;
+    const int64_t img = i >> 6, blk = img / groups;
+    const int g = (int)(img - blk * groups);
+    const int64_t src = (blk * 16 + rowpass_image_piece_row(l)) * SD + g * 64 + 16 * rowpass_image_piece_col(l);
+    auto pack = [&](const unsigned short* __restrict__ a) {
+        const v4u lo = *reinterpret_cast<const v4u*>(a + src), hi = *reinterpret_cast<const v4u*>(a + src + 8);
+        return v4u{__builtin_amdgcn_perm(lo.y, lo.x, 0x06040200u), __builtin_amdgcn_perm(lo.w, lo.z, 0x06040200u),
+                   __builtin_amdgcn_perm(hi.y, hi.x, 0x06040200u), __builtin_amdgcn_perm(hi.w, hi.z, 0x06040200u)};
+    };
+    *reinterpret_cast<v4u*>(X8 + i * 16) = pack(X16);
+    *reinterpret_cast<v4u*>(D8 + i * 16) = pack(D16);
+}
+
+hipError_t launch_build_rowpass_images(const unsigned short* X16, const unsigned short* D16, int64_t N16, int SD,
+                                       unsigned char* X8, unsigned char* D8, hipStream_t st) {
+    if (X16 == nullptr || D16 == nullptr || X8 == nullptr || D8 == nullptr || N16 < 16 || (N16 & 15) != 0 || SD < 64 || (SD & 63) != 0)
+        return hipErrorInvalidValue;
+    const int64_t pieces = N16 * SD / 16;
+    const int64_t grid = (pieces + 255) / 256;
+    if (grid > 0x7FFFFFFF) return hipErrorInvalidValue;
+    hipLaunchKernelGGL(k_build_rowpass_images, dim3((unsigned)grid), dim3(256), 0, st, X16, D16, SD, pieces, X8, D8);
+    return hipGetLastError();
+}
+
+size_t rowpass_v2_lds_bytes(int S, int n_u, int n_iter2, bool x16, bool pair = false, bool defer_c = false, bool bytes = false) {
     const int NW = (S + 63) / 64;
     const int maxw = NW <= 4 ? 4 : 8;
     const int nset = pair ? 2 : 1;
     const int nub = defer_c ? kDeferUbufSets : nset;
     const int nv = n_u * ((n_u + 2) & ~1);
     const size_t doubles = (size_t)((n_iter2 + 1) & ~1) + (size_t)nub * 16 * n_u + (size_t)nset * maxw * nv * 16 + maxw;
-    const int tile = defer_c ? kTileDBytes2 : (x16 ? kTileBytesX : kTileBytes2);
+    const int tile = bytes ? kTileDBytes8 : defer_c ? kTileDBytes2 : (x16 ? kTileBytesX : kTileBytes2);
     return doubles * sizeof(double) + (size_t)nset * NW * tile + (defer_c ? (size_t)NW * kRingBytes : 0);
 }
 
@@ -676,20 +739,23 @@
 }
 
 hipError_t launch_rowpass_v2(const ProblemView& p, const IterateView& it, int n_iter2, const UScratch& scratch, int* grid_out,
-                             bool pair, bool* paired_out, bool defer_c, bool* deferred_out, hipStream_t st) {
+                             bool pair, bool* paired_out, bool defer_c, bool* deferred_out, bool* bytes_out, hipStream_t st) {
     const int S = p.S, NW = (S + 63) / 64;
     pair = pair && p.X16 != nullptr && rowpass_v2_pair_fits(S, it.n_u, n_iter2);
     if (paired_out != nullptr) *paired_out = pair;
     defer_c = defer_c && pair && rowpass_v2_defer_fits(S, p.n_c, it.n_u, n_iter2);
     if (deferred_out != nullptr) *deferred_out = defer_c;
+    const bool bytes = defer_c && p.X8 != nullptr && p.D8 != nullptr;
+    if (bytes_out != nullptr) *bytes_out = bytes;
     return dispatch_int<0, 4>((p.n_c + 3) / 4, [&](auto nkc) {
         return dispatch_bool(p.X16 != nullptr, [&](auto xs) {
             return dispatch_int<1, 4>(it.n_u, [&](auto nu) {
-                const auto launch = [&](auto maxw, auto pair_t, auto defer_t) {
+                const auto launch = [&](auto maxw, auto pair_t, auto defer_t, auto bytes_t) {
                     constexpr int NU = decltype(nu)::value, MAXW = decltype(maxw)::value;
                     constexpr bool XS = decltype(xs)::value, PAIR = decltype(pair_t)::value, DEFER_C = decltype(defer_t)::value;
-                    constexpr auto kernel = k_rowpass_v2<decltype(nkc)::value, NU, MAXW, XS, PAIR, DEFER_C>;
-                    const size_t lds = rowpass_v2_lds_bytes(S, NU, n_iter2, XS, PAIR, DEFER_C);
+                    constexpr bool BYTES = decltype(bytes_t)::value;
+                    constexpr auto kernel = k_rowpass_v2<decltype(nkc)::value, NU, MAXW, XS, PAIR, DEFER_C, BYTES>;
+                    const size_t lds = rowpass_v2_lds_bytes(S, NU, n_iter2, XS, PAIR, DEFER_C, BYTES);
                     constexpr size_t kLdsCap = (size_t)(MAXW == 4 ? 80 : 160) * 1024;
                     if (NW > MAXW || (MAXW == 8 && NW <= 4) || (PAIR && NW < 2) || (DEFER_C && NW != 4) || lds > kLdsCap || p.N < 1 ||
                         p.SD < NW * 64 || (p.SD & 7) != 0 || p.ND < 1 || p.ND > 2)
@@ -700,7 +766,8 @@
                     }
                     const int grid = rowpass_v2_grid(p.N, S);
                     *grid_out = grid;
-                    hipLaunchKernelGGL(kernel, dim3(grid), dim3(NW * 64), lds, st, p.V, p.D16, p.X16, p.SD, p.Rtp, it.alpha,
+                    hipLaunchKernelGGL(kernel, dim3(grid), dim3(NW * 64), lds, st, p.V, BYTES ? reinterpret_cast<const unsigned short*>(p.D8) : p.D16,
+                                       BYTES ? reinterpret_cast<const unsigned short*>(p.X8) : p.X16, p.SD, p.Rtp, it.alpha,
                                        it.u, it.u_prev, it.state, p.N, S, p.n_c, n_iter2, it.mode, p.ND, scratch.slab,
                                        scratch.u2_partials
 #ifdef DMF_STAMPS
@@ -709,14 +776,15 @@
                                        );
                     return hipGetLastError();
                 };
-                if (S > 256) return launch(std::integral_constant<int, 8>{}, std::false_type{}, std::false_type{});
+                if (S > 256) return launch(std::integral_constant<int, 8>{}, std::false_type{}, std::false_type{}, std::false_type{});
                 if constexpr (decltype(xs)::value) {
                     if constexpr (rowpass_v2_defer_instance(decltype(nkc)::value, decltype(nu)::value)) {
-                        if (pair && defer_c) return launch(std::integral_constant<int, 4>{}, std::true_type{}, std::true_type{});
+                        if (pair && defer_c && bytes) return launch(std::integral_constant<int, 4>{}, std::true_type{}, std::true_type{}, std::true_type{});
+                        if (pair && defer_c) return launch(std::integral_constant<int, 4>{}, std::true_type{}, std::true_type{}, std::false_type{});
                     }
-                    if (pair) return launch(std::integral_constant<int, 4>{}, std::true_type{}, std::false_type{});
+                    if (pair) return launch(std::integral_constant<int, 4>{}, std::true_type{}, std::false_type{}, std::false_type{});
                 }
-                return launch(std::integral_constant<int, 4>{}, std::false_type{}, std::false_type{});
+                return launch(std::integral_constant<int, 4>{}, std::false_type{}, std::false_type{}, std::false_type{});
             });
         });
     });
diff --git a/demethify_amd/csrc/dmf_rowpass_image.h b/demethify_amd/csrc/dmf_rowpass_image.h
--- /dev/null
+++ b/demethify_amd/csrc/dmf_rowpass_image.h
@@ -0,0 +1,20 @@
+#pragma once
+
+#if defined(__HIPCC__) || defined(__CUDACC__)
+#define DMF_IMAGE_FN __host__ __device__ constexpr
+#else
+#define DMF_IMAGE_FN constexpr
+#endif
+
+namespace dmf {
+
+constexpr int kRowpassImageBytes = 16 * 64;
+
+DMF_IMAGE_FN int rowpass_image_dword(int row, int dword) {
+    return (4 * (row & 3) + (row >> 2)) * 16 + ((dword + 4 * (row & 3)) & 15);
+}
+DMF_IMAGE_FN int rowpass_image_byte(int row, int sample) { return 4 * rowpass_image_dword(row, sample >> 2) + (sample & 3); }
+DMF_IMAGE_FN int rowpass_image_piece_row(int piece) { return 4 * ((piece >> 2) & 3) + (piece >> 4); }
+DMF_IMAGE_FN int rowpass_image_piece_col(int piece) { return ((piece & 3) - ((piece >> 4) & 3)) & 3; }
+
+}
diff --git a/demethify_amd/csrc/dmf_select.h b/demethify_amd/csrc/dmf_select.h
--- a/demethify_amd/csrc/dmf_select.h
+++ b/demethify_amd/csrc/dmf_select.h
@@ -18,6 +18,7 @@
     bool x16 = false;
     bool rowpass_pair = true;
     bool rowpass_defer_c = true;
+    bool rowpass_bytes = true;
     bool x_byte = false;
     int level = 0;
     bool d_f32_exact = false;
diff --git a/demethify_amd/device.py b/demethify_amd/device.py
--- a/demethify_amd/device.py
+++ b/demethify_amd/device.py
@@ -90,6 +90,9 @@
 
     def set_rowpass_defer_c(self, enabled: bool):
         L.check(self._lib.dmf_context_set_rowpass_defer_c(self._h, int(bool(enabled))), "dmf_context_set_rowpass_defer_c")
+
+    def set_rowpass_bytes(self, enabled: bool):
+        L.check(self._lib.dmf_context_set_rowpass_bytes(self._h, int(bool(enabled))), "dmf_context_set_rowpass_bytes")
 
     def set_stop_confirmation(self, mode: int):
         L.check(self._lib.dmf_context_set_stop_confirmation(self._h, int(mode)), "dmf_context_set_stop_confirmation")
@@ -363,6 +366,18 @@
                 "dmf_problem_copy_out")
         return out
 
+    def has_byte_images(self) -> bool:
+        out = C.c_int()
+        L.check(self._lib.dmf_problem_has_byte_images(self._h, C.byref(out)), "dmf_problem_has_byte_images")
+        return bool(out.value)
+
+    def copy_out_image(self, name: str, report: dict | None = None) -> np.ndarray:
+        r = self.report() if report is None else report
+        out = np.empty((r["N16"] // 16, r["SD"] // 64, 1024), dtype=np.uint8)
+        L.check(self._lib.dmf_problem_copy_out(self._h, L.PROBLEM_BYTE_IMAGES[name], _ptr(out), out.nbytes),
+                "dmf_problem_copy_out")
+        return out
+
     def wls_intercept(self, u=None, target="v", host_arrays=None, f64_arrays=False):
         tg, u, n_u, flags = self._wls_args(u, target, f64_arrays)
         K = self.n_c + n_u
@@ -707,6 +722,11 @@
                 "dmf_solver_rowpass_launches")
         return total.value, paired.value
 
+    def rowpass_byte_launches(self):
+        n = C.c_int64()
+        L.check(self._lib.dmf_solver_rowpass_byte_launches(self._h, C.byref(n)), "dmf_solver_rowpass_byte_launches")
+        return n.value
+
     def rowpass_schedule_counts(self):
         total, paired, deferred = C.c_int64(), C.c_int64(), C.c_int64()
         L.check(self._lib.dmf_solver_rowpass_schedule_counts(self._h, C.byref(total), C.byref(paired), C.byref(deferred)),
diff --git a/include/demethify_hip.h b/include/demethify_hip.h
--- a/include/demethify_hip.h
+++ b/include/demethify_hip.h
@@ -63,6 +63,7 @@
 int dmf_context_set_x16(dmf_context* ctx, int enabled);
 int dmf_context_set_rowpass_pair(dmf_context* ctx, int enabled);
 int dmf_context_set_rowpass_defer_c(dmf_context* ctx, int enabled);
+int dmf_context_set_rowpass_bytes(dmf_context* ctx, int enabled);
 int dmf_context_set_stop_confirmation(dmf_context* ctx, int mode);
 
 int dmf_problem_create(dmf_context* ctx, int64_t N, int64_t S, int64_t n_c,
@@ -78,9 +79,11 @@
 int dmf_problem_gram_known(const dmf_problem* p, double* out, char* out_text, int64_t cap);
 enum { DMF_REPORT_INTS = 16, DMF_REPORT_DBLS = 8 };
 int dmf_problem_report(const dmf_problem* p, int64_t* out_ints, double* out_dbls);
+int dmf_problem_has_byte_images(const dmf_problem* p, int* out);
+int dmf_rowpass_image_offset(int row, int sample);
 enum {
     DMF_ARRAY_V = 0, DMF_ARRAY_D = 1, DMF_ARRAY_RT = 2, DMF_ARRAY_RTP = 3, DMF_ARRAY_D16 = 4, DMF_ARRAY_X16 = 5,
-    DMF_ARRAY_W16 = 6, DMF_ARRAY_DT8 = 7, DMF_ARRAY_MASK_BITS = 8, DMF_ARRAY_CONSTS = 9
+    DMF_ARRAY_W16 = 6, DMF_ARRAY_DT8 = 7, DMF_ARRAY_MASK_BITS = 8, DMF_ARRAY_CONSTS = 9, DMF_ARRAY_X8 = 10, DMF_ARRAY_D8 = 11
 };
 int dmf_problem_copy_out(const dmf_problem* p, int which, void* out, int64_t bytes);
 
@@ -152,6 +155,7 @@
                          double* last_stream_cost);
 int dmf_solver_rowpass_launches(const dmf_solver* s, int64_t* total, int64_t* paired);
 int dmf_solver_rowpass_schedule_counts(const dmf_solver* s, int64_t* total, int64_t* paired, int64_t* deferred);
+int dmf_solver_rowpass_byte_launches(const dmf_solver* s, int64_t* bytes);
 int dmf_solve(dmf_context* ctx, const dmf_problem* p, const double* u0, const double* alpha0,
               int64_t n_u, int mode, int64_t n_iter1, int64_t n_iter2, double tol, int flags,
               double* out_u, double* out_alpha, double* out_cost, int64_t* out_iters);
```

New measurement: 1947 outer iters/s (median of 6 runs). 5.1% higher.
